# benlevyx/vi-normflows

Hardware: AMD Instinct MI355X
Metric: ELBO samples/sec (whole node), 32-layer RealNVP on 784-dim synthetic (higher is better)
Workload: dtype bf16; 1 GPU; model=RealNVP-32 VI, 784-d, conditioner 392-1024-1024-784, 72.2M params, global_batch=65536, dim=784, parallelism=dp1

## Files before the change

csrc/bindings/gemm_ops.cpp:

```cpp
#include <vector>
#include <torch/library.h>
#include <ATen/ATen.h>

#include <cstdlib>

#include "bind_common.h"
#include "launchers.h"
#include "nf_common.h"

namespace {

long ld2(const at::Tensor& t) { return t.size(0) <= 1 ? t.size(1) : t.stride(0); }

void chk_amax_slots(const at::Tensor& t) {
  TORCH_CHECK(t.is_cuda() && t.scalar_type() == at::kFloat && t.is_contiguous() &&
                  t.numel() >= NF_AMAX_SLOTS,
              "amax_cur must hold ", NF_AMAX_SLOTS, " contiguous fp32 slots (ops.fp8.DelayedScale)");
}

void chk_mat(const at::Tensor& t, const char* n, at::ScalarType dt) {
  TORCH_CHECK(t.is_cuda(), n, " must be on the GPU");
  TORCH_CHECK(t.dim() == 2, n, " must be 2-D");
  TORCH_CHECK(t.scalar_type() == dt, n, " dtype ", t.scalar_type(), " expected ", dt);
  TORCH_CHECK(t.size(1) <= 1 || t.stride(1) == 1, n, " needs unit inner stride");
  TORCH_CHECK(ld2(t) % 8 == 0, n, " leading dimension must be a multiple of 8 (16-B rows)");
  TORCH_CHECK(reinterpret_cast<uintptr_t>(t.data_ptr()) % 16 == 0, n, " must be 16-B aligned");
}

void chk_q(const at::Tensor& t, const char* n) {
  TORCH_CHECK(t.is_cuda() && t.dim() == 2, n, " must be a 2-D GPU tensor");
  TORCH_CHECK(t.scalar_type() == at::kByte || t.scalar_type() == at::kFloat8_e4m3fn, n,
              " must be uint8 / float8_e4m3fn");
  TORCH_CHECK(t.stride(1) == 1 && ld2(t) % 16 == 0, n, " rows must be 16-B aligned");
  TORCH_CHECK(reinterpret_cast<uintptr_t>(t.data_ptr()) % 16 == 0, n, " must be 16-B aligned");
}

void chk_ranges(const at::Tensor& r, long ntiles, const char* n);

int64_t gemm_nt(const at::Tensor& x, const at::Tensor& W, const c10::optional<at::Tensor>& b,
                const at::Tensor& y, int64_t relu, const c10::optional<at::Tensor>& mask,
                bool mask_lanes) {
  chk_mat(x, "x", at::kBFloat16);
  chk_mat(W, "W", at::kBFloat16);
  chk_mat(y, "y", at::kBFloat16);
  const int M = x.size(0), K = x.size(1), N = W.size(0);
  TORCH_CHECK(W.size(1) == K, "W inner dim");
  TORCH_CHECK(y.size(0) == M && y.size(1) == N, "y shape");
  TORCH_CHECK(K % 32 == 0, "K must be a multiple of 32 (pad the operands)");
  TORCH_CHECK(N % 8 == 0, "N must be a multiple of 8");
  const void* bp = nullptr;
  if (b && b->defined()) {
    TORCH_CHECK(b->scalar_type() == at::kBFloat16 && b->numel() == N && b->is_contiguous(), "bias");
    bp = b->data_ptr();
  }
  void* mp = nullptr;
  long ldm = 0;
  if (mask && mask->defined()) {
    TORCH_CHECK(mask->is_cuda() && mask->dim() == 2 && mask->scalar_type() == at::kByte &&
                    mask->stride(1) == 1, "mask must be a 2-D uint8 GPU tensor with unit inner stride");
    TORCH_CHECK(relu, "the bitmask records 1(y > 0) of a ReLU layer");
    TORCH_CHECK(mask->size(0) == M && mask->size(1) * 8 == N, "mask shape [M, N/8]");
    TORCH_CHECK(ld2(y) % 8 == 0 && ((uintptr_t)y.data_ptr() & 15) == 0,
                "bitmask output needs 16-B aligned y rows");
    mp = mask->data_ptr();
    ldm = ld2(*mask);
  }
  if (mask_lanes) {
    TORCH_CHECK(mp, "mask_lanes needs a mask");
    if (!mask->is_contiguous()) return NF_LANES_SHAPE;
  }
  return nf_launch_gemm_nt(x.data_ptr(), ld2(x), W.data_ptr(), ld2(W), bp, y.data_ptr(), ld2(y), M,
                           N, K, (int)relu, cur_stream(), mp, ldm, mask_lanes ? 1 : 0);
}

int64_t gemm_mask_lanes_route(int64_t M, int64_t N, int64_t K_fwd, int64_t K_bwd, bool bwd_wt) {
  return nf_gemm_mask_lanes_route((int)M, (int)N, (int)K_fwd, (int)K_bwd, bwd_wt ? 1 : 0);
}

void gemm_nt_f32out(const at::Tensor& x, const at::Tensor& W, const at::Tensor& y) {
  chk_mat(x, "x", at::kBFloat16);
  chk_mat(W, "W", at::kBFloat16);
  chk_mat(y, "y", at::kFloat);
  const int M = x.size(0), K = x.size(1), N = W.size(0);
  TORCH_CHECK(W.size(1) == K, "W inner dim");
  TORCH_CHECK(y.size(0) == M && y.size(1) == N, "y shape");
  TORCH_CHECK(K % 32 == 0 && K > 0, "K must be a positive multiple of 32 (pad the operands)");
  TORCH_CHECK(N % 8 == 0, "N must be a multiple of 8");
  nf_launch_gemm_nt_f32out(x.data_ptr(), ld2(x), W.data_ptr(), ld2(W), y.data_ptr<float>(), ld2(y),
                           M, N, K, cur_stream());
}

void gemm_fp(const at::Tensor& A, bool a_kmajor, const at::Tensor& B, bool b_kmajor,
             const c10::optional<at::Tensor>& bias, const at::Tensor& C, bool accumulate,
             const c10::optional<at::Tensor>& dbias) {
  const auto dt = C.scalar_type();
  TORCH_CHECK(dt == at::kFloat || dt == at::kDouble, "gemm_fp: fp32 or fp64 output");
  auto chk = [&](const at::Tensor& t, const char* n) {
    TORCH_CHECK(t.is_cuda() && t.dim() == 2 && t.scalar_type() == dt, n,
                " must be a 2-D GPU tensor of the output's dtype");
    TORCH_CHECK(t.size(1) <= 1 || t.stride(1) == 1, n, " needs unit inner stride");
  };
  chk(A, "A"); chk(B, "B"); chk(C, "C");
  const int M = C.size(0), N = C.size(1);
  const int K = a_kmajor ? A.size(1) : A.size(0);
  TORCH_CHECK((a_kmajor ? A.size(0) : A.size(1)) == M, "A rows must match C rows");
  TORCH_CHECK((b_kmajor ? B.size(0) : B.size(1)) == N, "B rows must match C cols");
  TORCH_CHECK((b_kmajor ? B.size(1) : B.size(0)) == K, "A / B inner dims differ");
  const void* bp = nullptr;
  if (bias && bias->defined()) {
    TORCH_CHECK(bias->is_cuda() && bias->scalar_type() == dt && bias->is_contiguous() &&
                    bias->numel() == N, "bias: contiguous [N] of the output's dtype");
    bp = bias->data_ptr();
  }
  void* dbp = nullptr;
  if (dbias && dbias->defined()) {
    TORCH_CHECK(dbias->is_cuda() && dbias->scalar_type() == dt && dbias->is_contiguous() &&
                    dbias->numel() == M, "dbias: contiguous [M] of the output's dtype");
    dbp = dbias->data_ptr();
  }
  auto ld = [](const at::Tensor& t) { return t.size(0) <= 1 ? t.size(1) : t.stride(0); };
  const int S = nf_gemm_fp_splits(M, N, K);
  at::Tensor work;
  if (S > 1) work = at::empty({(long)S * ((long)M * N + M)}, C.options());
  nf_launch_gemm_fp(dt == at::kDouble, A.data_ptr(), ld(A), a_kmajor, B.data_ptr(), ld(B),
                    b_kmajor, bp, C.data_ptr(), ld(C), dbp, M, N, K, accumulate, cur_stream(),
                    S > 1 ? work.data_ptr() : nullptr, S);
}

int64_t gemm_nn(const at::Tensor& dy, const at::Tensor& W, const c10::optional<at::Tensor>& h,
                const at::Tensor& dx, bool accumulate, const c10::optional<at::Tensor>& hbits,
                const c10::optional<at::Tensor>& Wt, bool hbits_lanes) {
  chk_mat(dy, "dy", at::kBFloat16);
  chk_mat(W, "W", at::kBFloat16);
  const bool f32 = dx.scalar_type() == at::kFloat;
  chk_mat(dx, "dx", f32 ? at::kFloat : at::kBFloat16);
  const int M = dy.size(0), K = dy.size(1), N = W.size(1);
  TORCH_CHECK(W.size(0) == K, "W rows must equal dy cols");
  const bool use_wt = Wt && Wt->defined();
  if (use_wt) {
    chk_mat(*Wt, "Wt", at::kBFloat16);
    TORCH_CHECK(Wt->size(0) == N && Wt->size(1) == K, "Wt must be W^T [N, K]");
    TORCH_CHECK(!f32 && !accumulate, "the transposed-weight path writes bf16");
    TORCH_CHECK(ld2(*Wt) % 8 == 0 && ((uintptr_t)Wt->data_ptr() & 15) == 0, "Wt rows 16-B");
  }
  TORCH_CHECK(dx.size(0) == M && dx.size(1) == N, "dx shape");
  TORCH_CHECK(K % 32 == 0 && N % 8 == 0, "K % 32 and N % 8 required");
  const void* hp = nullptr;
  long ldh = 0;
  if (h && h->defined()) {
    TORCH_CHECK(!f32, "ReLU-mask epilogue writes bf16");
    chk_mat(*h, "h", at::kBFloat16);
    TORCH_CHECK(h->size(0) == M && h->size(1) == N, "h shape");
    hp = h->data_ptr();
    ldh = ld2(*h);
  }
  int bits = 0;
  if (hbits && hbits->defined()) {
    TORCH_CHECK(!hp, "pass either h or hbits");
    TORCH_CHECK(!f32, "ReLU-mask epilogue writes bf16");
    TORCH_CHECK(hbits->is_cuda() && hbits->dim() == 2 && hbits->scalar_type() == at::kByte &&
                    hbits->stride(1) == 1, "hbits must be a 2-D uint8 GPU tensor with unit inner stride");
    TORCH_CHECK(hbits->size(0) == M && hbits->size(1) * 8 == N, "hbits shape [M, N/8]");
    hp = hbits->data_ptr();
    ldh = ld2(*hbits);
    bits = 1;
    if (hbits_lanes) {
      if (!hbits->is_contiguous()) return NF_LANES_SHAPE;
      bits = 2;
    }
  }
  TORCH_CHECK(!hbits_lanes || bits, "hbits_lanes needs hbits");
  TORCH_CHECK(!accumulate || f32, "accumulate needs an fp32 output");
  if (use_wt)
    return nf_launch_gemm256_nt_dgrad(dy.data_ptr(), ld2(dy), Wt->data_ptr(), ld2(*Wt), hp, ldh,
                                      bits, dx.data_ptr(), ld2(dx), M, N, K, cur_stream());
  return nf_launch_gemm_nn(dy.data_ptr(), ld2(dy), W.data_ptr(), ld2(W), hp, ldh, dx.data_ptr(),
                           ld2(dx), f32, accumulate, M, N, K, cur_stream(), bits);
}

void transpose_bf16_batched(const at::Tensor& desc, int64_t n, int64_t tiles) {
  TORCH_CHECK(desc.is_cuda() && desc.scalar_type() == at::kLong && desc.is_contiguous() &&
                  desc.numel() >= 5 * n, "desc: int64 GPU [n, 5]");
  nf_launch_transpose_bf16_batched(desc.data_ptr(), (int)n, (int)tiles, cur_stream());
}

void gemm_tn(const at::Tensor& dy, const at::Tensor& x, const at::Tensor& dW,
             const c10::optional<at::Tensor>& db) {
  chk_mat(dy, "dy", at::kBFloat16);
  chk_mat(x, "x", at::kBFloat16);
  chk_mat(dW, "dW", at::kFloat);
  const int K = dy.size(0), M = dy.size(1), N = x.size(1);
  TORCH_CHECK(x.size(0) == K, "batch mismatch");
  TORCH_CHECK(dW.size(0) == M && dW.size(1) == N, "dW shape");
  TORCH_CHECK(K % 32 == 0 && M % 8 == 0 && N % 8 == 0, "K % 32, M % 8, N % 8 required");
  float* dbp = nullptr;
  if (db && db->defined()) {
    TORCH_CHECK(db->scalar_type() == at::kFloat && db->numel() == M && db->is_contiguous(), "db");
    dbp = db->data_ptr<float>();
  }
  const int splits = nf_gemm_tn_splits(M, N, K);
  at::Tensor work;
  float* wp = nullptr;
  const long ws = nf_gemm_tn_workspace(M, N, splits);
  if (ws > 0) {
    work = at::empty({ws}, dW.options());
    wp = work.data_ptr<float>();
  }
  nf_launch_gemm_tn(dy.data_ptr(), ld2(dy), x.data_ptr(), ld2(x), dW.data_ptr<float>(), ld2(dW), dbp,
                    M, N, K, splits, wp, cur_stream());
}

void gemm_tn_group(at::TensorList dy, at::TensorList x, at::TensorList dW,
                   const c10::List<c10::optional<at::Tensor>>& db,
                   const c10::List<c10::optional<at::Tensor>>& skip,
                   const c10::List<c10::optional<at::Tensor>>& cmask) {
  const size_t n = dy.size();
  TORCH_CHECK(n >= 1 && n <= 4 && x.size() == n && dW.size() == n && db.size() == n,
              "gemm_tn_group: 1..4 problems with matching lists");
  NfTnProblem pr[4];
  for (size_t p = 0; p < n; ++p) {
    chk_mat(dy[p], "dy", at::kBFloat16);
    chk_mat(x[p], "x", at::kBFloat16);
    chk_mat(dW[p], "dW", at::kFloat);
    const int K = dy[p].size(0), M = dy[p].size(1), N = x[p].size(1);
    TORCH_CHECK(x[p].size(0) == K, "batch mismatch");
    TORCH_CHECK(dW[p].size(0) == M && dW[p].size(1) == N, "dW shape");
    TORCH_CHECK(K % 32 == 0 && M % 8 == 0 && N % 8 == 0, "K % 32, M % 8, N % 8 required");
    float* dbp = nullptr;
    const c10::optional<at::Tensor> b = db.get(p);
    if (b && b->defined()) {
      TORCH_CHECK(b->scalar_type() == at::kFloat && b->numel() == M && b->is_contiguous(), "db");
      dbp = b->data_ptr<float>();
    }
    pr[p] = NfTnProblem{dy[p].data_ptr(), ld2(dy[p]), x[p].data_ptr(), ld2(x[p]),
                        dW[p].data_ptr<float>(), ld2(dW[p]), dbp, M, N, K};
    if (skip.size() == n) {
      const c10::optional<at::Tensor> sk = skip.get(p);
      if (sk && sk->defined()) {
        TORCH_CHECK(sk->is_cuda() && sk->scalar_type() == at::kByte && sk->is_contiguous() &&
                        sk->numel() == (long)((M + 127) / 128) * ((N + 127) / 128), "skip flags");
        pr[p].skip = sk->data_ptr<uint8_t>();
      }
    }
    if (cmask.size() == n) {
      const c10::optional<at::Tensor> cm = cmask.get(p);
      if (cm && cm->defined()) {
        TORCH_CHECK(cm->is_cuda() && cm->scalar_type() == at::kByte && cm->is_contiguous() &&
                        cm->numel() == (long)M * N && N % 4 == 0, "cmask [M,N] uint8");
        TORCH_CHECK(ld2(dW[p]) == N, "cmask needs a dense dW");
        pr[p].cmask = cm->data_ptr<uint8_t>();
      }
    }
  }
  at::Tensor work;
  float* wp = nullptr;
  const long ws = nf_gemm_tn_group_workspace((int)n, pr);
  if (ws > 0) {
    work = at::empty({ws}, dW[0].options());
    wp = work.data_ptr<float>();
  }
  nf_launch_gemm_tn_group((int)n, pr, wp, cur_stream());
}

static void gemm_tn_multi_impl(at::TensorList dy, at::TensorList x, at::TensorList dW,
                               const c10::List<c10::optional<at::Tensor>>& db, int64_t tile0,
                               int64_t ntiles, const c10::List<c10::optional<at::Tensor>>& tiles,
                               const c10::List<c10::optional<at::Tensor>>& cmask,
                               const at::Tensor* f8_scales, at::IntArrayRef sa_idx,
                               at::IntArrayRef sb_idx, int layout = 0) {
  const size_t n = dy.size();
  TORCH_CHECK(layout >= 0 && layout <= 4 && (layout == 0 || !f8_scales), "layout 0..4, bf16");
  const bool f8 = f8_scales != nullptr;
  const auto odt = f8 ? at::kFloat8_e4m3fn : at::kBFloat16;
  if (f8) {
    TORCH_CHECK(f8_scales->is_cuda() && f8_scales->scalar_type() == at::kFloat &&
                    f8_scales->is_contiguous() && sa_idx.size() == n && sb_idx.size() == n,
                "gemm_tn_multi_f8: fp32 scale pool and one (sa, sb) index pair per problem");
    for (size_t p = 0; p < n; ++p)
      TORCH_CHECK(sa_idx[p] >= 0 && sb_idx[p] >= 0 && sa_idx[p] < f8_scales->numel() &&
                      sb_idx[p] < f8_scales->numel() && sa_idx[p] <= 0xffff &&
                      sb_idx[p] <= 0x7fff,
                  "gemm_tn_multi_f8: scale index outside the pool");
  }
  TORCH_CHECK(n >= 1 && n <= 40 && x.size() == n && dW.size() == n && db.size() == n,
              "gemm_tn_multi: 1..40 problems with matching lists");
  TORCH_CHECK((tiles.size() == 0 || tiles.size() == n) && (cmask.size() == 0 || cmask.size() == n),
              "gemm_tn_multi: tiles / cmask lists must be empty or one entry per problem");
  std::vector<NfTnProblem> pr(n);
  long total = 0;
  for (size_t p = 0; p < n; ++p) {
    chk_mat(dy[p], "dy", odt);
    chk_mat(x[p], "x", odt);
    chk_mat(dW[p], "dW", at::kFloat);
    const int K = layout == 2 ? dy[p].size(1) : dy[p].size(0);
    const int M = layout == 2 ? dy[p].size(0) : dy[p].size(1);
    const int N = layout == 1 ? x[p].size(0) : x[p].size(1);
    TORCH_CHECK((layout == 1 ? x[p].size(1) : x[p].size(0)) == K, "batch mismatch");
    TORCH_CHECK(dW[p].size(0) == M && dW[p].size(1) == N, "dW shape");
    TORCH_CHECK(K % 32 == 0 && M % 8 == 0 && N % 8 == 0, "K % 32, M % 8, N % 8 required");
    TORCH_CHECK(!f8 || (K % 128 == 0 && M % 16 == 0 && N % 16 == 0 && ld2(dy[p]) % 16 == 0 &&
                        ld2(x[p]) % 16 == 0 && ld2(dW[p]) % 4 == 0 &&
                        ((uintptr_t)dW[p].data_ptr() & 15) == 0),
                "gemm_tn_multi_f8: K % 128, M / N / ld % 16, 16-B aligned dW");
    TORCH_CHECK(ld2(dy[p]) < (1L << 31) && ld2(x[p]) < (1L << 31) && ld2(dW[p]) < (1L << 31),
                "leading dimensions must fit in int32");
    float* dbp = nullptr;
    const c10::optional<at::Tensor> b = db.get(p);
    if (b && b->defined()) {
      TORCH_CHECK(b->scalar_type() == at::kFloat && b->numel() == M && b->is_contiguous(), "db");
      dbp = b->data_ptr<float>();
    }
    pr[p] = NfTnProblem{dy[p].data_ptr(), ld2(dy[p]), x[p].data_ptr(), ld2(x[p]),
                        dW[p].data_ptr<float>(), ld2(dW[p]), dbp, M, N, K};
    if (f8) {
      pr[p].sa_idx = (int)sa_idx[p];
      pr[p].sb_idx = (int)sb_idx[p];
    }
    int nt = nf_gemm256_tiles(M, N);
    if (tiles.size() == n) {
      const c10::optional<at::Tensor> tl = tiles.get(p);
      if (tl && tl->defined()) {
        TORCH_CHECK(tl->is_cuda() && tl->scalar_type() == at::kShort && tl->is_contiguous() &&
                        tl->numel() >= 1 && tl->numel() <= nt,
                    "tiles: int16 GPU list of active 256x256 tile ids");
        pr[p].tiles = reinterpret_cast<const unsigned short*>(tl->data_ptr<int16_t>());
        pr[p].ntiles_active = nt = (int)tl->numel();
      }
    }
    if (cmask.size() == n) {
      const c10::optional<at::Tensor> cm = cmask.get(p);
      if (cm && cm->defined()) {
        TORCH_CHECK(cm->is_cuda() && cm->scalar_type() == at::kByte && cm->is_contiguous() &&
                        cm->numel() == (long)M * N && ld2(dW[p]) == N, "cmask [M,N] uint8, dense dW");
        pr[p].cmask = cm->data_ptr<uint8_t>();
      }
    }
    total += nt;
  }
  TORCH_CHECK(tile0 >= 0 && ntiles >= 1 && tile0 + ntiles <= total, "tile range outside the ",
              total, " tiles of the problem list");
  nf_launch_gemm256_tn_multi((int)n, pr.data(), (int)tile0, (int)ntiles, cur_stream(),
                             f8 ? f8_scales->data_ptr<float>() : nullptr, layout);
}

void gemm_tn_multi_layout(at::TensorList dy, at::TensorList x, at::TensorList dW,
                          const c10::List<c10::optional<at::Tensor>>& db, int64_t tile0,
                          int64_t ntiles, int64_t layout) {
  const c10::List<c10::optional<at::Tensor>> none;
  gemm_tn_multi_impl(dy, x, dW, db, tile0, ntiles, none, none, nullptr, {}, {}, (int)layout);
}

void gemm_tn_multi(at::TensorList dy, at::TensorList x, at::TensorList dW,
                   const c10::List<c10::optional<at::Tensor>>& db, int64_t tile0, int64_t ntiles,
                   const c10::List<c10::optional<at::Tensor>>& tiles,
                   const c10::List<c10::optional<at::Tensor>>& cmask) {
  gemm_tn_multi_impl(dy, x, dW, db, tile0, ntiles, tiles, cmask, nullptr, {}, {});
}

void gemm_tn_multi_f8(at::TensorList dy, at::TensorList x, at::TensorList dW,
                      const c10::List<c10::optional<at::Tensor>>& db, int64_t tile0,
                      int64_t ntiles, const c10::List<c10::optional<at::Tensor>>& tiles,
                      const c10::List<c10::optional<at::Tensor>>& cmask, const at::Tensor& scales,
                      at::IntArrayRef sa_idx, at::IntArrayRef sb_idx) {
  gemm_tn_multi_impl(dy, x, dW, db, tile0, ntiles, tiles, cmask, &scales, sa_idx, sb_idx);
}

void fp8_colsum(at::TensorList q, at::TensorList out, const at::Tensor& scales,
                at::IntArrayRef sidx, const at::Tensor& part) {
  const size_t n = q.size();
  TORCH_CHECK(n >= 1 && n <= 40 && out.size() == n && sidx.size() == n,
              "fp8_colsum: 1..40 tensors with matching lists");
  TORCH_CHECK(scales.is_cuda() && scales.scalar_type() == at::kFloat && scales.is_contiguous(),
              "fp8_colsum: fp32 scale pool");
  std::vector<const void*> qp(n);
  std::vector<long> ld(n);
  std::vector<int> K(n), N(n), si(n);
  std::vector<float*> op(n);
  for (size_t i = 0; i < n; ++i) {
    chk_mat(q[i], "q", at::kFloat8_e4m3fn);
    K[i] = (int)q[i].size(0);
    N[i] = (int)q[i].size(1);
    TORCH_CHECK(out[i].is_cuda() && out[i].scalar_type() == at::kFloat && out[i].is_contiguous() &&
                    out[i].numel() == N[i], "fp8_colsum: out[i] fp32 [N]");
    TORCH_CHECK(sidx[i] >= 0 && sidx[i] < scales.numel(), "fp8_colsum: scale index");
    qp[i] = q[i].data_ptr();
    ld[i] = ld2(q[i]);
    op[i] = out[i].data_ptr<float>();
    si[i] = (int)sidx[i];
  }
  TORCH_CHECK(part.is_cuda() && part.scalar_type() == at::kFloat && part.is_contiguous() &&
                  part.numel() >= nf_fp8_colsum_workspace((int)n, N.data()),
              "fp8_colsum: part workspace too small");
  nf_launch_fp8_colsum((int)n, qp.data(), ld.data(), K.data(), N.data(), op.data(), si.data(),
                       scales.data_ptr<float>(), part.data_ptr<float>(), cur_stream());
}

void gemm_nt_cpl(const at::Tensor& h, const at::Tensor& W, const c10::optional<at::Tensor>& b,
                 const c10::optional<at::Tensor>& st_opt, const at::Tensor& x, const at::Tensor& y,
                 const c10::optional<at::Tensor>& yb, const at::Tensor& ldjp, bool ldj_init,
                 double scale, bool inverse) {
  chk_mat(h, "h", at::kBFloat16);
  chk_mat(W, "W", at::kBFloat16);
  const int M = h.size(0), K = h.size(1), Dh = x.size(1);
  const bool has_st = st_opt && st_opt->defined();
  TORCH_CHECK(has_st || inverse, "st (s_hat output) is required in the forward");
  if (has_st) {
    chk_mat(*st_opt, "st", at::kBFloat16);
    TORCH_CHECK(st_opt->size(0) == M && st_opt->size(1) >= Dh, "st shape");
  }
  TORCH_CHECK(W.size(1) == K && W.size(0) >= 2 * Dh, "W: [>= 2 Dh, K]");
  TORCH_CHECK(K % 32 == 0 && Dh % 8 == 0, "K % 32 and Dh % 8 required");
  for (const at::Tensor* t : {&x, &y})
    TORCH_CHECK(t->is_cuda() && t->scalar_type() == at::kFloat && t->dim() == 2 &&
                    t->stride(1) == 1 && t->size(0) == M && t->size(1) == Dh &&
                    ld2(*t) % 4 == 0 && reinterpret_cast<uintptr_t>(t->data_ptr()) % 16 == 0,
                "x, y: fp32 [M, Dh], 16-B aligned rows");
  const int ntn = (Dh + 127) / 128;
  TORCH_CHECK(ldjp.is_cuda() && ldjp.scalar_type() == at::kFloat && ldjp.dim() == 2 &&
                  ldjp.size(0) >= ntn && ldjp.size(1) == M && ldjp.stride(1) == 1,
              "ldjp: fp32 [ceil(Dh/128), M]");
  const void* bp = nullptr;
  if (b && b->defined()) {
    TORCH_CHECK(b->scalar_type() == at::kBFloat16 && b->numel() == W.size(0) && b->is_contiguous(),
                "bias");
    bp = b->data_ptr();
  }
  void* ybp = nullptr;
  long ldyb = 0;
  int ybw = 0;
  if (yb && yb->defined()) {
    chk_mat(*yb, "yb", at::kBFloat16);
    TORCH_CHECK(yb->size(0) == M && yb->size(1) >= Dh && yb->size(1) % 8 == 0, "yb shape");
    ybp = yb->data_ptr();
    ldyb = ld2(*yb);
    ybw = (int)yb->size(1);
  }
  nf_launch_gemm256_nt_cpl(h.data_ptr(), ld2(h), W.data_ptr(), ld2(W), (int)W.size(0), bp,
                           has_st ? st_opt->data_ptr() : nullptr, has_st ? ld2(*st_opt) : 0, M,
                           K, Dh, x.data_ptr<float>(), ld2(x), y.data_ptr<float>(), ld2(y), ybp,
                           ldyb, ybw, ldjp.data_ptr<float>(), ldjp.stride(0), ldj_init,
                           (float)scale, cur_stream(), inverse ? 1 : 0);
}

void gemm_nn_cpl(const at::Tensor& dy, const at::Tensor& W, const at::Tensor& G,
                 const at::Tensor& s_hat, const at::Tensor& x, const at::Tensor& dst,
                 const at::Tensor& gx, double scale, double c, const c10::optional<at::Tensor>& Wt) {
  chk_mat(dy, "dy", at::kBFloat16);
  chk_mat(W, "W", at::kBFloat16);
  const int M = dy.size(0), K = dy.size(1), N = W.size(1);
  TORCH_CHECK(W.size(0) == K, "W rows must equal dy cols");
  const bool use_wt = Wt && Wt->defined();
  if (use_wt) {
    chk_mat(*Wt, "Wt", at::kBFloat16);
    TORCH_CHECK(Wt->size(0) == N && Wt->size(1) == K, "Wt must be W^T [N, K]");
    TORCH_CHECK(ld2(*Wt) % 8 == 0 && ((uintptr_t)Wt->data_ptr() & 15) == 0, "Wt rows 16-B");
  }
  TORCH_CHECK(K % 32 == 0 && N % 8 == 0, "K % 32 and N % 8 required");
  for (const at::Tensor* t : {&G, &s_hat, &x, &dst, &gx})
    TORCH_CHECK(t->is_cuda() && t->dim() == 2 && t->stride(1) == 1 && t->size(0) == M,
                "gemm_nn_cpl: 2-D GPU operands with unit inner stride and M rows");
  const int Dh = x.size(1);
  const bool x_bf16 = x.scalar_type() == at::kBFloat16;
  const bool g_bf16 = G.scalar_type() == at::kBFloat16, gx_bf16 = gx.scalar_type() == at::kBFloat16;
  TORCH_CHECK((G.scalar_type() == at::kFloat || (g_bf16 && x_bf16)) && G.size(1) == N,
              "G: fp32 (or bf16 with bf16 x) [M, N]");
  TORCH_CHECK((x.scalar_type() == at::kFloat || (x_bf16 && use_wt)) &&
                  (gx.scalar_type() == at::kFloat || (gx_bf16 && x_bf16)) && gx.size(1) == Dh,
              "x: fp32 (or bf16 with Wt) [M, Dh], gx: fp32 (or bf16 with bf16 x) [M, Dh]");
  TORCH_CHECK(s_hat.scalar_type() == at::kBFloat16 && s_hat.size(1) >= Dh, "s_hat: bf16 [M, >= Dh]");
  TORCH_CHECK(dst.scalar_type() == at::kBFloat16 && dst.size(1) >= 2 * Dh && dst.size(1) <= Dh + N,
              "dst: bf16 [M, 2 Dh .. Dh + N]");
  auto al = [](const at::Tensor& t, uintptr_t a) {
    return reinterpret_cast<uintptr_t>(t.data_ptr()) % a == 0;
  };
  TORCH_CHECK(Dh % 4 == 0 && N % 4 == 0 && ld2(G) % 4 == 0 && ld2(x) % 4 == 0 &&
                  ld2(gx) % 4 == 0 && ld2(dst) % 4 == 0 && ld2(s_hat) % 4 == 0,
              "gemm_nn_cpl: Dh, N and every leading dimension must be multiples of 4");
  TORCH_CHECK(al(G, g_bf16 ? 8 : 16) && al(x, x_bf16 ? 8 : 16) && al(gx, gx_bf16 ? 8 : 16) &&
                  al(dst, 8) && al(s_hat, 8),
              "gemm_nn_cpl: G / x / gx must be 16-B aligned (8-B as bf16), dst / s_hat 8-B aligned");
  nf_launch_gemm256_nn_cpl(dy.data_ptr(), ld2(dy), use_wt ? Wt->data_ptr() : W.data_ptr(),
                           use_wt ? ld2(*Wt) : ld2(W), (const float*)G.data_ptr(),
                           ld2(G), M, N, K, s_hat.data_ptr(), ld2(s_hat), (const float*)x.data_ptr(),
                           ld2(x), dst.data_ptr(), ld2(dst), (int)dst.size(1),
                           (float*)gx.data_ptr(), ld2(gx), Dh, (float)scale, (float)c, cur_stream(),
                           use_wt ? 1 : 0, nullptr, 1, 0, nullptr, x_bf16 ? 1 : 0, g_bf16 ? 1 : 0,
                           gx_bf16 ? 1 : 0);
}

void maf_gemm_fwd(const at::Tensor& h, const c10::optional<at::Tensor>& hs, const at::Tensor& W,
                  const c10::optional<at::Tensor>& ws, const c10::optional<at::Tensor>& b,
                  const at::Tensor& krange, const at::Tensor& s_out, const at::Tensor& x,
                  const c10::optional<at::Tensor>& u, const c10::optional<at::Tensor>& ubf,
                  const at::Tensor& ldjp,
                  bool ldj_init, double bound, const c10::optional<at::Tensor>& uq,
                  const c10::optional<at::Tensor>& q_amax_prev,
                  const c10::optional<at::Tensor>& q_scale,
                  const c10::optional<at::Tensor>& q_amax_cur) {
  const bool f8 = h.scalar_type() != at::kBFloat16;
  if (f8) {
    chk_q(h, "h");
    chk_q(W, "W");
    TORCH_CHECK(hs && hs->defined() && ws && ws->defined(), "fp8 operands need hs and ws");
    TORCH_CHECK(hs->is_cuda() && hs->scalar_type() == at::kFloat && hs->numel() >= 1, "hs");
    TORCH_CHECK(ws->is_cuda() && ws->scalar_type() == at::kFloat && ws->is_contiguous() &&
                    ws->numel() == W.size(0), "ws: fp32 [2D]");
  } else {
    chk_mat(h, "h", at::kBFloat16);
    chk_mat(W, "W", at::kBFloat16);
  }
  chk_mat(s_out, "s_out", at::kBFloat16);
  const bool x_bf16 = x.scalar_type() == at::kBFloat16;
  chk_mat(x, "x", x_bf16 ? at::kBFloat16 : at::kFloat);
  const bool has_u = u && u->defined();
  if (has_u) chk_mat(*u, "u", at::kFloat);
  TORCH_CHECK(has_u || (ubf && ubf->defined()),
              "maf_gemm_fwd: u may be omitted only with a ubf output (a bf16 state)");
  const int M = h.size(0), K = h.size(1), D = x.size(1);
  TORCH_CHECK(W.size(0) == 2 * D && W.size(1) == K, "W must be [2D, K]");
  TORCH_CHECK(K % (f8 ? 128 : 32) == 0, "maf_gemm_fwd: K must be a multiple of 32 (e4m3: 128)");
  TORCH_CHECK(D % 128 == 0 && x.size(0) == M && (!has_u || (u->size(0) == M && u->size(1) == D)) &&
                  s_out.size(0) == M && s_out.size(1) == D, "maf_gemm_fwd shapes (D % 128 == 0)");
  chk_ranges(krange, D / 128, "krange");
  TORCH_CHECK(ldjp.is_cuda() && ldjp.scalar_type() == at::kFloat && ldjp.dim() == 2 &&
                  ldjp.size(0) >= D / 128 && ldjp.size(1) == M && ldjp.stride(1) == 1,
              "ldjp: fp32 [D/128, M]");
  const void* bp = nullptr;
  if (b && b->defined()) {
    TORCH_CHECK(b->scalar_type() == at::kBFloat16 && b->numel() == 2 * D && b->is_contiguous(),
                "b: bf16 [2D]");
    bp = b->data_ptr();
  }
  void* ubp = nullptr;
  long ldub = 0;
  if (ubf && ubf->defined()) {
    chk_mat(*ubf, "ubf", at::kBFloat16);
    TORCH_CHECK(ubf->size(0) == M && ubf->size(1) == D, "ubf shape");
    ubp = ubf->data_ptr();
    ldub = ld2(*ubf);
  }
  void* qp = nullptr;
  long ldq = 0;
  const float* qap = nullptr;
  float* qs = nullptr;
  float* qac = nullptr;
  if (uq && uq->defined()) {
    TORCH_CHECK(f8, "the e4m3 copy of u belongs to the fp8 path");
    chk_q(*uq, "uq");
    TORCH_CHECK(uq->size(0) == M && uq->size(1) == D, "uq shape");
    TORCH_CHECK(q_amax_prev && q_scale && q_amax_cur, "uq needs the delayed-scale state");
    chk_amax_slots(*q_amax_cur);
    qp = uq->data_ptr();
    ldq = ld2(*uq);
    qap = q_amax_prev->data_ptr<float>();
    qs = q_scale->data_ptr<float>();
    qac = q_amax_cur->data_ptr<float>();
  }
  nf_launch_gemm256_maf_fwd(h.data_ptr(), ld2(h), f8 ? 1 : 0, f8 ? hs->data_ptr<float>() : nullptr,
                            W.data_ptr(), ld2(W), f8 ? ws->data_ptr<float>() : nullptr, bp,
                            krange.data_ptr<int>(), s_out.data_ptr(), ld2(s_out), M, K, D,
                            (const float*)x.data_ptr(), ld2(x),
                            has_u ? u->data_ptr<float>() : nullptr, has_u ? ld2(*u) : 0, ubp, ldub,
                            ldjp.data_ptr<float>(), ldjp.stride(0), ldj_init, (float)bound, qp, ldq,
                            qap, qs, qac, cur_stream(), x_bf16 ? 1 : 0);
}

struct F8Out {
  void* q = nullptr;
  long ldq = 0;
  const float* ap = nullptr;
  float* qs = nullptr;
  float* ac = nullptr;
};
F8Out f8_out(const c10::optional<at::Tensor>& q, const c10::optional<at::Tensor>& amax_prev,
             const c10::optional<at::Tensor>& scale, const c10::optional<at::Tensor>& amax_cur,
             long rows, long cols) {
  F8Out o;
  if (!(q && q->defined())) return o;
  chk_q(*q, "q");
  TORCH_CHECK(q->size(0) == rows && q->size(1) == cols, "e4m3 copy shape");
  TORCH_CHECK(amax_prev && scale && amax_cur && amax_prev->defined() && scale->defined() &&
                  amax_cur->defined(), "the e4m3 copy needs the delayed-scale state");
  chk_amax_slots(*amax_cur);
  o.q = q->data_ptr();
  o.ldq = ld2(*q);
  o.ap = amax_prev->data_ptr<float>();
  o.qs = scale->data_ptr<float>();
  o.ac = amax_cur->data_ptr<float>();
  return o;
}

void chk_scales(const c10::optional<at::Tensor>& sa, const c10::optional<at::Tensor>& sb,
                long nb) {
  TORCH_CHECK(sa && sa->defined() && sb && sb->defined(), "fp8 operands need sa and sb");
  TORCH_CHECK(sa->is_cuda() && sa->scalar_type() == at::kFloat && sa->numel() >= 1, "sa");
  TORCH_CHECK(sb->is_cuda() && sb->scalar_type() == at::kFloat && sb->is_contiguous() &&
                  sb->numel() == nb && ((uintptr_t)sb->data_ptr() & 15) == 0,
              "sb: fp32 per-row scales, 16-B aligned");
}

void fp8_dgrad(const at::Tensor& dyq, const at::Tensor& sa, const at::Tensor& Wtq,
               const at::Tensor& sb, const at::Tensor& h, const c10::optional<at::Tensor>& dx_opt,
               const at::Tensor& krange256, const c10::optional<at::Tensor>& dxq,
               const c10::optional<at::Tensor>& q_amax_prev,
               const c10::optional<at::Tensor>& q_scale,
               const c10::optional<at::Tensor>& q_amax_cur) {
  chk_q(dyq, "dyq");
  chk_q(Wtq, "Wtq");
  const int M = dyq.size(0), K = dyq.size(1), N = Wtq.size(0);
  TORCH_CHECK(Wtq.size(1) == K && K % 128 == 0 && N % 8 == 0, "Wtq [N, K], K % 128 == 0");
  const bool h_bits = h.scalar_type() == at::kByte;
  if (h_bits) {
    TORCH_CHECK(h.is_cuda() && h.dim() == 2 && h.size(0) == M && h.size(1) * 8 >= N &&
                    h.stride(1) == 1, "h bitmask: uint8 [M, N/8]");
  } else {
    chk_mat(h, "h", at::kBFloat16);
  }
  TORCH_CHECK(h.size(0) == M && (h_bits || h.size(1) == N), "h");
  const bool has_dx = dx_opt && dx_opt->defined();
  TORCH_CHECK(has_dx || (dxq && dxq->defined()), "fp8_dgrad: dx and / or dxq");
  if (has_dx) {
    chk_mat(*dx_opt, "dx", at::kBFloat16);
    TORCH_CHECK(dx_opt->size(0) == M && dx_opt->size(1) == N, "dx");
  }
  chk_scales(sa, sb, N);
  const long nt = (N + 255) / 256;
  const int segs = krange256.numel() == 4 * nt ? 2 : 1;
  chk_ranges(krange256, segs * nt, "krange256");
  const F8Out o = f8_out(dxq, q_amax_prev, q_scale, q_amax_cur, M, N);
  nf_launch_gemm256_fp8_dgrad(dyq.data_ptr(), ld2(dyq), sa.data_ptr<float>(), Wtq.data_ptr(),
                              ld2(Wtq), sb.data_ptr<float>(), h.data_ptr(), ld2(h), h_bits ? 1 : 0,
                              has_dx ? dx_opt->data_ptr() : nullptr, has_dx ? ld2(*dx_opt) : N,
                              M, N, K, krange256.data_ptr<int>(), segs,
                              o.q, o.ldq, o.ap, o.qs, o.ac, cur_stream());
}

void maf_gemm_bwd(const at::Tensor& dy, const at::Tensor& Wt, const at::Tensor& krange256,
                  const at::Tensor& G, const at::Tensor& s_raw, const at::Tensor& u,
                  const c10::optional<at::Tensor>& dst_opt, const at::Tensor& gx, double bound,
                  double c,
                  const c10::optional<at::Tensor>& sa, const c10::optional<at::Tensor>& sb,
                  const c10::optional<at::Tensor>& dstq,
                  const c10::optional<at::Tensor>& q_amax_prev,
                  const c10::optional<at::Tensor>& q_scale,
                  const c10::optional<at::Tensor>& q_amax_cur) {
  const bool f8 = dy.scalar_type() != at::kBFloat16;
  if (f8) {
    chk_q(dy, "dy");
    chk_q(Wt, "Wt");
    chk_scales(sa, sb, Wt.size(0));
  } else {
    chk_mat(dy, "dy", at::kBFloat16);
    chk_mat(Wt, "Wt", at::kBFloat16);
    TORCH_CHECK(!(dstq && dstq->defined()), "the e4m3 copy of dst belongs to the fp8 path");
  }
  chk_mat(s_raw, "s_raw", at::kBFloat16);
  const bool has_dst = dst_opt && dst_opt->defined();
  TORCH_CHECK(has_dst || (f8 && dstq && dstq->defined()), "maf_gemm_bwd: dst and / or dstq");
  if (has_dst) chk_mat(*dst_opt, "dst", at::kBFloat16);
  chk_mat(G, "G", at::kFloat);
  const bool u_bf16 = u.scalar_type() == at::kBFloat16;
  chk_mat(u, "u", u_bf16 ? at::kBFloat16 : at::kFloat);
  chk_mat(gx, "gx", at::kFloat);
  const int M = dy.size(0), K = dy.size(1), D = Wt.size(0);
  TORCH_CHECK(Wt.size(1) == K && K % 32 == 0 && D % 8 == 0, "Wt must be [D, K], K % 32 == 0");
  TORCH_CHECK(!f8 || K % 128 == 0, "maf_gemm_bwd: e4m3 operands need K % 128 == 0");
  for (const at::Tensor* t : {&G, &s_raw, &u, &gx})
    TORCH_CHECK(t->size(0) == M && t->size(1) == D, "G / s_raw / u / gx: [M, D]");
  TORCH_CHECK(!has_dst || (dst_opt->size(0) == M && dst_opt->size(1) == 2 * D),
              "dst: bf16 [M, 2D]");
  const long nt = (D + 255) / 256;
  const int segs = krange256.numel() == 4 * nt ? 2 : 1;
  chk_ranges(krange256, segs * nt, "krange256");
  NfF8Operands fo{};
  if (f8) {
    const F8Out o = f8_out(dstq, q_amax_prev, q_scale, q_amax_cur, M, 2 * D);
    fo.sa = sa->data_ptr<float>();
    fo.sb = sb->data_ptr<float>();
    fo.q = o.q; fo.ldq = o.ldq;
    fo.q_amax_prev = o.ap; fo.q_scale_out = o.qs; fo.q_amax_cur = o.ac;
  }
  nf_launch_gemm256_nn_cpl(dy.data_ptr(), ld2(dy), Wt.data_ptr(), ld2(Wt), G.data_ptr<float>(),
                           ld2(G), M, D, K, s_raw.data_ptr(), ld2(s_raw),
                           (const float*)u.data_ptr(), ld2(u),
                           has_dst ? dst_opt->data_ptr() : nullptr,
                           has_dst ? ld2(*dst_opt) : 2 * D, 2 * D, gx.data_ptr<float>(), ld2(gx),
                           D, (float)bound, (float)c, cur_stream(), 1, krange256.data_ptr<int>(),
                           segs, 1, f8 ? &fo : nullptr, u_bf16 ? 1 : 0);
}

void fp8_quant_rows_strided(const at::Tensor& x, int64_t layer_stride, int64_t rows_per,
                            int64_t layers, int64_t C, const at::Tensor& q, const at::Tensor& scale) {
  TORCH_CHECK(x.is_cuda() && (x.scalar_type() == at::kFloat || x.scalar_type() == at::kBFloat16) &&
                  x.is_contiguous(), "x fp32 / bf16 GPU");
  TORCH_CHECK(x.numel() >= (layers - 1) * layer_stride + rows_per * C, "x too small");
  chk_q(q, "q");
  TORCH_CHECK(q.size(0) == rows_per * layers && q.size(1) >= C && q.size(1) % 4 == 0, "q shape");
  TORCH_CHECK(scale.is_cuda() && scale.scalar_type() == at::kFloat &&
                  scale.numel() == rows_per * layers, "scale");
  nf_launch_fp8_quant_rows_strided(x.data_ptr(), x.scalar_type() == at::kBFloat16, C,
                                   layer_stride, (int)rows_per,
                                   (int)(rows_per * layers), (int)C, q.data_ptr(), ld2(q), q.size(1),
                                   scale.data_ptr<float>(), cur_stream());
}

void maf_fwd(const at::Tensor& x, const at::Tensor& o, double bound, const at::Tensor& u,
             const c10::optional<at::Tensor>& ubf, const c10::optional<at::Tensor>& uq,
             const c10::optional<at::Tensor>& amax_prev, const c10::optional<at::Tensor>& scale,
             const c10::optional<at::Tensor>& amax_cur, const at::Tensor& ldj, bool ldj_init) {
  chk_mat(x, "x", at::kFloat);
  chk_mat(o, "o", at::kBFloat16);
  chk_mat(u, "u", at::kFloat);
  const int B = x.size(0), D = x.size(1);
  TORCH_CHECK(D % 4 == 0 && o.size(0) == B && o.size(1) == 2 * D && u.size(0) == B && u.size(1) == D,
              "maf_fwd shapes");
  TORCH_CHECK(ldj.is_cuda() && ldj.scalar_type() == at::kFloat && ldj.numel() == B, "ldj");
  void* ub = nullptr;
  long ldub = 0;
  if (ubf && ubf->defined()) {
    chk_mat(*ubf, "ubf", at::kBFloat16);
    ub = ubf->data_ptr();
    ldub = ld2(*ubf);
  }
  void* q = nullptr;
  long ldq = 0;
  const float* ap = nullptr;
  float* sc = nullptr;
  float* ac = nullptr;
  if (uq && uq->defined()) {
    chk_q(*uq, "uq");
    TORCH_CHECK(amax_prev && scale && amax_cur, "fp8 output needs the delayed-scale state");
    q = uq->data_ptr();
    ldq = ld2(*uq);
    ap = amax_prev->data_ptr<float>();
    sc = scale->data_ptr<float>();
    ac = amax_cur->data_ptr<float>();
    chk_amax_slots(*amax_cur);
  }
  nf_launch_maf_fwd(x.data_ptr<float>(), ld2(x), o.data_ptr(), ld2(o), B, D, (float)bound,
                    u.data_ptr<float>(), ld2(u), ub, ldub, q, ldq, ap, sc, ac,
                    ldj.data_ptr<float>(), ldj_init, cur_stream());
}

void maf_bwd(const at::Tensor& gu, const at::Tensor& u, const at::Tensor& o, double bound,
             double c_ldj, const at::Tensor& dout, const at::Tensor& gx,
             const c10::optional<at::Tensor>& c_row) {
  chk_mat(gu, "gu", at::kFloat);
  chk_mat(u, "u", at::kFloat);
  chk_mat(o, "o", at::kBFloat16);
  chk_mat(dout, "dout", at::kBFloat16);
  chk_mat(gx, "gx", at::kFloat);
  const int B = gu.size(0), D = gu.size(1);
  TORCH_CHECK(D % 4 == 0 && u.size(0) == B && u.size(1) == D && o.size(0) == B &&
                  (o.size(1) == 2 * D || o.size(1) == D) && dout.size(1) == 2 * D &&
                  gx.size(1) == D, "maf_bwd shapes");
  const void* sp = static_cast<const at::BFloat16*>(o.data_ptr()) + (o.size(1) == 2 * D ? D : 0);
  const float* cr = nullptr;
  if (c_row && c_row->defined()) {
    TORCH_CHECK(c_row->is_cuda() && c_row->scalar_type() == at::kFloat &&
                    c_row->is_contiguous() && c_row->numel() == B, "c_row: fp32 [B]");
    cr = c_row->data_ptr<float>();
  }
  nf_launch_maf_bwd(gu.data_ptr<float>(), ld2(gu), u.data_ptr<float>(), ld2(u), sp,
                    ld2(o), B, D, (float)bound, (float)c_ldj, dout.data_ptr(), ld2(dout),
                    gx.data_ptr<float>(), ld2(gx), cur_stream(), cr);
}

void iaf_gate_fwd(const at::Tensor& o, const at::Tensor& z, double gate_bias, const at::Tensor& y,
                  const at::Tensor& ldj, const c10::optional<at::Tensor>& ybf) {
  chk_mat(o, "o", at::kBFloat16);
  chk_mat(z, "z", at::kFloat);
  chk_mat(y, "y", at::kFloat);
  const int B = z.size(0), D = z.size(1);
  TORCH_CHECK(D % 4 == 0 && o.size(0) == B && o.size(1) == 2 * D && y.size(0) == B &&
                  y.size(1) == D, "iaf_gate_fwd shapes");
  TORCH_CHECK(ldj.is_cuda() && ldj.scalar_type() == at::kFloat && ldj.is_contiguous() &&
                  ldj.numel() == B, "ldj: fp32 [B]");
  void* yb = nullptr;
  long ldyb = 0;
  if (ybf && ybf->defined()) {
    chk_mat(*ybf, "ybf", at::kBFloat16);
    TORCH_CHECK(ybf->size(0) == B && ybf->size(1) == D && ld2(*ybf) % 4 == 0 &&
                    reinterpret_cast<uintptr_t>(ybf->data_ptr()) % 8 == 0,
                "ybf: bf16 [B, D], 8-B aligned rows");
    yb = ybf->data_ptr();
    ldyb = ld2(*ybf);
  }
  nf_launch_iaf_gate_fwd(o.data_ptr(), ld2(o), z.data_ptr<float>(), ld2(z), B, D, (float)gate_bias,
                         y.data_ptr<float>(), ld2(y), ldj.data_ptr<float>(), cur_stream(), yb,
                         ldyb);
}

void iaf_gate_bwd(const at::Tensor& gy, const c10::optional<at::Tensor>& gl, const at::Tensor& z,
                  const at::Tensor& o, double gate_bias, const at::Tensor& dout,
                  const at::Tensor& gz) {
  chk_mat(gy, "gy", at::kFloat);
  chk_mat(z, "z", at::kFloat);
  chk_mat(o, "o", at::kBFloat16);
  chk_mat(dout, "dout", at::kBFloat16);
  chk_mat(gz, "gz", at::kFloat);
  const int B = z.size(0), D = z.size(1);
  TORCH_CHECK(D % 4 == 0 && gy.size(0) == B && gy.size(1) == D && o.size(0) == B &&
                  o.size(1) == 2 * D && dout.size(0) == B && dout.size(1) == 2 * D &&
                  gz.size(0) == B && gz.size(1) == D, "iaf_gate_bwd shapes");
  const float* glp = nullptr;
  if (gl && gl->defined()) {
    TORCH_CHECK(gl->is_cuda() && gl->scalar_type() == at::kFloat && gl->is_contiguous() &&
                    gl->numel() == B, "gl: fp32 [B]");
    glp = gl->data_ptr<float>();
  }
  nf_launch_iaf_gate_bwd(gy.data_ptr<float>(), ld2(gy), glp, z.data_ptr<float>(), ld2(z),
                         o.data_ptr(), ld2(o), B, D, (float)gate_bias, dout.data_ptr(), ld2(dout),
                         gz.data_ptr<float>(), ld2(gz), cur_stream());
}

void chk_ranges(const at::Tensor& r, long ntiles, const char* n) {
  TORCH_CHECK(r.is_cuda() && r.scalar_type() == at::kInt && r.is_contiguous() && r.numel() == 2 * ntiles,
              n, " must be an int32 GPU tensor [n_tiles, 2]");
}

void masked_gemm_nt(const at::Tensor& x, const at::Tensor& W, const c10::optional<at::Tensor>& b,
                    const at::Tensor& y, int64_t relu, const at::Tensor& krange,
                    const c10::optional<at::Tensor>& krange256) {
  chk_mat(x, "x", at::kBFloat16);
  chk_mat(W, "W", at::kBFloat16);
  chk_mat(y, "y", at::kBFloat16);
  const int M = x.size(0), K = x.size(1), N = W.size(0);
  TORCH_CHECK(W.size(1) == K && y.size(0) == M && y.size(1) == N, "shapes");
  TORCH_CHECK(K % 32 == 0 && N % 8 == 0, "K % 32 and N % 8 required");
  chk_ranges(krange, (N + 127) / 128, "krange");
  const void* bp = (b && b->defined()) ? b->data_ptr() : nullptr;
  const int* k256 = nullptr;
  if (krange256 && krange256->defined()) {
    chk_ranges(*krange256, (N + 255) / 256, "krange256");
    k256 = krange256->data_ptr<int>();
  }
  nf_launch_gemm_nt_masked(x.data_ptr(), ld2(x), W.data_ptr(), ld2(W), bp, y.data_ptr(), ld2(y), M,
                           N, K, (int)relu, krange.data_ptr<int>(), cur_stream(), k256);
}

void masked_gemm_nn(const at::Tensor& dy, const at::Tensor& W, const c10::optional<at::Tensor>& h,
                    const at::Tensor& dx, const at::Tensor& krange, bool accumulate,
                    const c10::optional<at::Tensor>& krange256, const c10::optional<at::Tensor>& Wt) {
  chk_mat(dy, "dy", at::kBFloat16);
  chk_mat(W, "W", at::kBFloat16);
  const bool f32 = dx.scalar_type() == at::kFloat;
  chk_mat(dx, "dx", f32 ? at::kFloat : at::kBFloat16);
  const int M = dy.size(0), K = dy.size(1), N = W.size(1);
  TORCH_CHECK(W.size(0) == K && dx.size(0) == M && dx.size(1) == N, "shapes");
  TORCH_CHECK(K % 32 == 0 && N % 8 == 0, "K % 32 and N % 8 required");
  chk_ranges(krange, (N + 127) / 128, "krange");
  const void* hp = nullptr;
  long ldh = 0;
  if (h && h->defined()) {
    chk_mat(*h, "h", at::kBFloat16);
    hp = h->data_ptr();
    ldh = ld2(*h);
  }
  TORCH_CHECK(!accumulate || f32, "accumulate needs an fp32 dx");
  const int* k256 = nullptr;
  int segs = 1;
  if (krange256 && krange256->defined()) {
    const long nt = (N + 255) / 256;
    segs = krange256->numel() == 4 * nt ? 2 : 1;
    chk_ranges(*krange256, segs * nt, "krange256");
    TORCH_CHECK(!hp || (ld2(*h) % 8 == 0 && ((uintptr_t)hp & 15) == 0),
                "ReLU-mask operand rows must be 16-B aligned for the 256x256 kernel");
    k256 = krange256->data_ptr<int>();
  }
  const void* wtp = nullptr;
  long ldwt = 0;
  if (Wt && Wt->defined()) {
    chk_mat(*Wt, "Wt", at::kBFloat16);
    TORCH_CHECK(Wt->size(0) == N && Wt->size(1) == K, "Wt must be W^T [N, K]");
    TORCH_CHECK(ld2(*Wt) % 8 == 0 && ((uintptr_t)Wt->data_ptr() & 15) == 0, "Wt rows 16-B");
    wtp = Wt->data_ptr();
    ldwt = ld2(*Wt);
  }
  nf_launch_gemm_nn_masked(dy.data_ptr(), ld2(dy), W.data_ptr(), ld2(W), hp, ldh, dx.data_ptr(),
                           ld2(dx), f32, accumulate, M, N, K, krange.data_ptr<int>(), cur_stream(),
                           k256, segs, wtp, ldwt);
}

void masked_gemm_tn(const at::Tensor& dy, const at::Tensor& x, const at::Tensor& dW,
                    const c10::optional<at::Tensor>& db, const at::Tensor& skip) {
  chk_mat(dy, "dy", at::kBFloat16);
  chk_mat(x, "x", at::kBFloat16);
  chk_mat(dW, "dW", at::kFloat);
  const int K = dy.size(0), M = dy.size(1), N = x.size(1);
  TORCH_CHECK(x.size(0) == K && dW.size(0) == M && dW.size(1) == N, "shapes");
  TORCH_CHECK(K % 32 == 0 && M % 8 == 0 && N % 8 == 0, "K % 32, M % 8, N % 8 required");
  TORCH_CHECK(skip.is_cuda() && skip.scalar_type() == at::kByte && skip.is_contiguous() &&
                  skip.numel() == (long)((M + 127) / 128) * ((N + 127) / 128),
              "skip must be a uint8 GPU tensor [tiles]");
  float* dbp = (db && db->defined()) ? db->data_ptr<float>() : nullptr;
  const int splits = nf_gemm_tn_splits(M, N, K);
  at::Tensor work;
  float* wp = nullptr;
  const long ws = nf_gemm_tn_workspace(M, N, splits);
  if (ws > 0) {
    work = at::empty({ws}, dW.options());
    wp = work.data_ptr<float>();
  }
  nf_launch_gemm_tn_masked(dy.data_ptr(), ld2(dy), x.data_ptr(), ld2(x), dW.data_ptr<float>(),
                           ld2(dW), dbp, M, N, K, splits, wp, skip.data_ptr<unsigned char>(),
                           cur_stream());
}

}


void fp8_quant_rows(const at::Tensor& x, const at::Tensor& q, const at::Tensor& scale) {
  TORCH_CHECK(x.is_cuda() && x.dim() == 2 && x.stride(1) == 1, "x: 2-D GPU, unit inner stride");
  TORCH_CHECK(x.scalar_type() == at::kBFloat16 || x.scalar_type() == at::kFloat, "x bf16/fp32");
  chk_q(q, "q");
  TORCH_CHECK(q.size(0) == x.size(0) && q.size(1) >= x.size(1) && q.size(1) % 4 == 0, "q shape");
  TORCH_CHECK(scale.is_cuda() && scale.scalar_type() == at::kFloat && scale.numel() == x.size(0) &&
                  scale.is_contiguous(), "scale [rows] fp32");
  nf_launch_fp8_quant_rows(x.data_ptr(), x.scalar_type() == at::kBFloat16, ld2(x), x.size(0),
                           x.size(1), q.data_ptr(), ld2(q), q.size(1), scale.data_ptr<float>(),
                           cur_stream());
}

void fp8_quant_tensor(const at::Tensor& x, const at::Tensor& q, const at::Tensor& amax_prev,
                      const at::Tensor& scale, const at::Tensor& amax_cur) {
  TORCH_CHECK(x.is_cuda() && x.dim() == 2 && x.stride(1) == 1, "x: 2-D GPU, unit inner stride");
  TORCH_CHECK(x.scalar_type() == at::kBFloat16 || x.scalar_type() == at::kFloat, "x bf16/fp32");
  chk_q(q, "q");
  TORCH_CHECK(q.size(0) == x.size(0) && q.size(1) >= x.size(1) && q.size(1) % 4 == 0, "q shape");
  for (const at::Tensor* t : {&amax_prev, &scale, &amax_cur})
    TORCH_CHECK(t->is_cuda() && t->scalar_type() == at::kFloat && t->numel() >= 1, "scalars fp32");
  chk_amax_slots(amax_cur);
  nf_launch_fp8_quant_tensor(x.data_ptr(), x.scalar_type() == at::kBFloat16, ld2(x), x.size(0),
                             x.size(1), q.data_ptr(), ld2(q), q.size(1), amax_prev.data_ptr<float>(),
                             scale.data_ptr<float>(), amax_cur.data_ptr<float>(), cur_stream());
}

void gemm_fp8_nt(const at::Tensor& xq, const at::Tensor& sx, const at::Tensor& wq,
                 const at::Tensor& sw, const c10::optional<at::Tensor>& b,
                 const c10::optional<at::Tensor>& y_opt, int64_t relu,
                 const c10::optional<at::Tensor>& krange,
                 const c10::optional<at::Tensor>& yq, const c10::optional<at::Tensor>& q_amax_prev,
                 const c10::optional<at::Tensor>& q_scale, const c10::optional<at::Tensor>& q_amax_cur,
                 const c10::optional<at::Tensor>& krange256,
                 const c10::optional<at::Tensor>& mask_out) {
  chk_q(xq, "xq");
  chk_q(wq, "wq");
  const bool has_y = y_opt && y_opt->defined();
  const bool has_mask = mask_out && mask_out->defined();
  const int M = xq.size(0), K = xq.size(1), N = wq.size(0);
  TORCH_CHECK(wq.size(1) == K, "shapes");
  if (has_y) {
    chk_mat(*y_opt, "y", at::kBFloat16);
    TORCH_CHECK(y_opt->size(0) == M && y_opt->size(1) == N, "y shape");
  }
  TORCH_CHECK(has_y || (yq && yq->defined()) || has_mask, "gemm_fp8_nt: no output");
  if (has_mask) {
    TORCH_CHECK(mask_out->is_cuda() && mask_out->scalar_type() == at::kByte && mask_out->dim() == 2 &&
                    mask_out->size(0) == M && mask_out->size(1) * 8 >= N && mask_out->stride(1) == 1 &&
                    relu, "mask_out: uint8 [M, N/8] bitmask of a ReLU product");
  }
  TORCH_CHECK(K % 128 == 0 && N % 8 == 0, "K % 128 and N % 8 required");
  TORCH_CHECK(sx.is_cuda() && sx.scalar_type() == at::kFloat && (sx.numel() == M || sx.numel() == 1) &&
                  sx.is_contiguous(), "sx [M] or [1]");
  TORCH_CHECK(sw.is_cuda() && sw.scalar_type() == at::kFloat && sw.numel() == N && sw.is_contiguous(), "sw");
  const void* bp = nullptr;
  if (b && b->defined()) {
    TORCH_CHECK(b->scalar_type() == at::kBFloat16 && b->numel() == N && b->is_contiguous(), "bias");
    bp = b->data_ptr();
  }
  const int* kr = nullptr;
  if (krange && krange->defined()) {
    chk_ranges(*krange, (N + 127) / 128, "krange");
    kr = krange->data_ptr<int>();
  }
  void* qp = nullptr;
  long ldq = 0;
  const float* qap = nullptr;
  float* qs = nullptr;
  float* qac = nullptr;
  if (yq && yq->defined()) {
    chk_q(*yq, "yq");
    TORCH_CHECK(yq->size(0) == M && yq->size(1) == N, "yq shape");
    TORCH_CHECK(q_amax_prev && q_scale && q_amax_cur, "yq needs the delayed-scale state");
    qp = yq->data_ptr();
    ldq = ld2(*yq);
    qap = q_amax_prev->data_ptr<float>();
    qs = q_scale->data_ptr<float>();
    qac = q_amax_cur->data_ptr<float>();
    chk_amax_slots(*q_amax_cur);
  }
  const bool dense = !(krange && krange->defined());
  const bool has256 = krange256 && krange256->defined();
  const long ldy = has_y ? ld2(*y_opt) : N;
  const bool lean = !has_y || has_mask;
  if ((dense || has256) && (lean || nf_gemm_prefer_256(M, N, K)) && ld2(xq) % 16 == 0 &&
      ld2(wq) % 16 == 0 && ldy % 8 == 0 && (!qp || ldq % 8 == 0)) {
    const int* k256 = nullptr;
    if (has256) {
      chk_ranges(*krange256, (N + 255) / 256, "krange256");
      k256 = krange256->data_ptr<int>();
    }
    nf_launch_gemm256_fp8_nt(xq.data_ptr(), ld2(xq), sx.data_ptr<float>(),
                             sx.numel() == M && M > 1, wq.data_ptr(), ld2(wq), sw.data_ptr<float>(),
                             bp, has_y ? y_opt->data_ptr() : nullptr, ldy, M, N, K, (int)relu,
                             k256, qp, ldq, qap, qs, qac, cur_stream(),
                             has_mask ? mask_out->data_ptr<uint8_t>() : nullptr,
                             has_mask ? ld2(*mask_out) : 0);
    return;
  }
  TORCH_CHECK(!lean, "gemm_fp8_nt: y-less / bitmask forms need the 256 kernel (krange256, 16-B rows)");
  nf_launch_gemm_fp8_nt(xq.data_ptr(), ld2(xq), sx.data_ptr<float>(), sx.numel() == M && M > 1,
                        wq.data_ptr(), ld2(wq),
                        sw.data_ptr<float>(), bp, y_opt->data_ptr(), ldy, M, N, K, (int)relu, kr,
                        qp, ldq, qap, qs, qac, cur_stream());
}

int64_t gemm_set_mode(int64_t mode) { return nf_gemm_set_mode((int)mode); }
int64_t gemm_pair(int64_t mode) { return nf_gemm256_set_pair((int)mode); }
int nf_gemm_cpl4w(int on);
int64_t gemm_cpl4w(int64_t on) { return nf_gemm_cpl4w((int)on); }
int nf_gemm256_xcd_pack(int on);
int64_t gemm_wgrad_xcd_pack(int64_t on) { return nf_gemm256_xcd_pack((int)on); }
int64_t gemm_persist(int64_t on) {
  const int prev = nf_gemm256_get_persist();
  if (on >= 0) nf_gemm256_set_persist((int)on);
  return prev;
}
int64_t gemm_grid_reserve(int64_t cus) {
  return nf_gemm256_set_reserve((int)cus);
}
#ifdef NF_G256_STAMPS
void nf_g256_set_stamps(void* p);
void g256_set_stamps(const at::Tensor& buf) { nf_g256_set_stamps(buf.numel() ? buf.data_ptr() : nullptr); }
#endif

TORCH_LIBRARY_FRAGMENT(vinf, m) {
#ifdef NF_G256_STAMPS
  m.def("g256_set_stamps(Tensor buf) -> ()", &g256_set_stamps);
#endif
  m.def("gemm_set_mode(int mode) -> int", &gemm_set_mode);
  m.def("gemm_pair(int mode) -> int", &gemm_pair);
  m.def("gemm_cpl4w(int on) -> int", &gemm_cpl4w);
  m.def("gemm_persist(int on) -> int", &gemm_persist);
  m.def("gemm_grid_reserve(int cus) -> int", &gemm_grid_reserve);
  m.def("gemm_wgrad_xcd_pack(int on) -> int", &gemm_wgrad_xcd_pack);
  m.def("fp8_quant_rows(Tensor x, Tensor(a!) q, Tensor(b!) scale) -> ()");
  m.def("fp8_quant_tensor(Tensor x, Tensor(a!) q, Tensor amax_prev, Tensor(b!) scale, Tensor(c!) amax_cur) -> ()");
  m.def("gemm_fp8_nt(Tensor xq, Tensor sx, Tensor wq, Tensor sw, Tensor? b, Tensor(a!)? y, int relu, Tensor? krange, Tensor(b!)? yq=None, Tensor? q_amax_prev=None, Tensor(c!)? q_scale=None, Tensor(d!)? q_amax_cur=None, Tensor? krange256=None, Tensor(e!)? mask_out=None) -> ()");
  m.def("masked_gemm_nt(Tensor x, Tensor W, Tensor? b, Tensor(a!) y, int relu, Tensor krange, Tensor? krange256=None) -> ()");
  m.def("masked_gemm_nn(Tensor dy, Tensor W, Tensor? h, Tensor(a!) dx, Tensor krange, bool accumulate=False, Tensor? krange256=None, Tensor? Wt=None) -> ()");
  m.def("masked_gemm_tn(Tensor dy, Tensor x, Tensor(a!) dW, Tensor(b!)? db, Tensor skip) -> ()");
  m.def("gemm_nt(Tensor x, Tensor W, Tensor? b, Tensor(a!) y, int relu, Tensor(b!)? mask=None, bool mask_lanes=False) -> int");
  m.def("gemm_mask_lanes_route(int M, int N, int K_fwd, int K_bwd, bool bwd_wt) -> int", &gemm_mask_lanes_route);
  m.def("gemm_nt_f32out(Tensor x, Tensor W, Tensor(a!) y) -> ()");
  m.def("gemm_fp(Tensor A, bool a_kmajor, Tensor B, bool b_kmajor, Tensor? bias, Tensor(a!) C, bool accumulate, Tensor(b!)? dbias=None) -> ()");
  m.def("gemm_nn(Tensor dy, Tensor W, Tensor? h, Tensor(a!) dx, bool accumulate, Tensor? hbits=None, Tensor? Wt=None, bool hbits_lanes=False) -> int");
  m.def("transpose_bf16_batched(Tensor desc, int n, int tiles) -> ()");
  m.def("gemm_tn(Tensor dy, Tensor x, Tensor(a!) dW, Tensor(b!)? db) -> ()");
  m.def("gemm_tn_group(Tensor[] dy, Tensor[] x, Tensor(a!)[] dW, Tensor(b!)?[] db, Tensor?[] skip, Tensor?[] cmask) -> ()");
  m.def("gemm_tn_multi(Tensor[] dy, Tensor[] x, Tensor(a!)[] dW, Tensor(b!)?[] db, int tile0, int ntiles, Tensor?[] tiles, Tensor?[] cmask) -> ()");
  m.def("gemm_tn_multi_layout(Tensor[] dy, Tensor[] x, Tensor(a!)[] dW, Tensor(b!)?[] db, int tile0, int ntiles, int layout) -> ()");
  m.def("fp8_colsum(Tensor[] q, Tensor(a!)[] out, Tensor scales, int[] sidx, Tensor(b!) part) -> ()");
  m.def("gemm_tn_multi_f8(Tensor[] dy, Tensor[] x, Tensor(a!)[] dW, Tensor(b!)?[] db, int tile0, int ntiles, Tensor?[] tiles, Tensor?[] cmask, Tensor scales, int[] sa_idx, int[] sb_idx) -> ()");
  m.def("gemm_nt_cpl(Tensor h, Tensor W, Tensor? b, Tensor(a!)? st, Tensor x, Tensor(b!) y, Tensor(c!)? yb, Tensor(d!) ldjp, bool ldj_init, float scale, bool inverse=False) -> ()");
  m.def("gemm_nn_cpl(Tensor dy, Tensor W, Tensor G, Tensor s_hat, Tensor x, Tensor(a!) dst, Tensor(b!) gx, float scale, float c, Tensor? Wt=None) -> ()");
  m.def("maf_gemm_fwd(Tensor h, Tensor? hs, Tensor W, Tensor? ws, Tensor? b, Tensor krange, Tensor(a!) s_out, Tensor x, Tensor(b!)? u, Tensor(c!)? ubf, Tensor(d!) ldjp, bool ldj_init, float bound, Tensor(e!)? uq=None, Tensor? q_amax_prev=None, Tensor(f!)? q_scale=None, Tensor(g!)? q_amax_cur=None) -> ()");
  m.def("maf_gemm_bwd(Tensor dy, Tensor Wt, Tensor krange256, Tensor G, Tensor s_raw, Tensor u, Tensor(a!)? dst, Tensor(b!) gx, float bound, float c, Tensor? sa=None, Tensor? sb=None, Tensor(c!)? dstq=None, Tensor? q_amax_prev=None, Tensor(d!)? q_scale=None, Tensor(e!)? q_amax_cur=None) -> ()");
  m.def("fp8_dgrad(Tensor dyq, Tensor sa, Tensor Wtq, Tensor sb, Tensor h, Tensor(a!)? dx, Tensor krange256, Tensor(b!)? dxq=None, Tensor? q_amax_prev=None, Tensor(c!)? q_scale=None, Tensor(d!)? q_amax_cur=None) -> ()");
  m.def("fp8_quant_rows_strided(Tensor x, int layer_stride, int rows_per, int layers, int C, Tensor(a!) q, Tensor(b!) scale) -> ()");
  m.def("maf_fwd(Tensor x, Tensor o, float bound, Tensor(a!) u, Tensor(b!)? ubf, Tensor(c!)? uq, Tensor? amax_prev, Tensor(d!)? scale, Tensor(e!)? amax_cur, Tensor(f!) ldj, bool ldj_init) -> ()");
  m.def("iaf_gate_fwd(Tensor o, Tensor z, float gate_bias, Tensor(a!) y, Tensor(b!) ldj, "
        "Tensor(c!)? ybf=None) -> ()");
  m.def("iaf_gate_bwd(Tensor gy, Tensor? gl, Tensor z, Tensor o, float gate_bias, Tensor(a!) dout, Tensor(b!) gz) -> ()");
  m.def("maf_bwd(Tensor gu, Tensor u, Tensor o, float bound, float c_ldj, Tensor(a!) dout, Tensor(b!) gx, Tensor? c_row=None) -> ()");
}

TORCH_LIBRARY_IMPL(vinf, CUDA, m) {
  m.impl("masked_gemm_nt", &masked_gemm_nt);
  m.impl("masked_gemm_nn", &masked_gemm_nn);
  m.impl("masked_gemm_tn", &masked_gemm_tn);
  m.impl("gemm_nt", &gemm_nt);
  m.impl("gemm_nt_f32out", &gemm_nt_f32out);
  m.impl("gemm_fp", &gemm_fp);
  m.impl("gemm_nn", &gemm_nn);
  m.impl("transpose_bf16_batched", &transpose_bf16_batched);
  m.impl("gemm_tn", &gemm_tn);
  m.impl("gemm_tn_group", &gemm_tn_group);
  m.impl("gemm_tn_multi", &gemm_tn_multi);
  m.impl("gemm_tn_multi_f8", &gemm_tn_multi_f8);
  m.impl("fp8_colsum", &fp8_colsum);
  m.impl("gemm_tn_multi_layout", &gemm_tn_multi_layout);
  m.impl("gemm_nn_cpl", &gemm_nn_cpl);
  m.impl("gemm_nt_cpl", &gemm_nt_cpl);
  m.impl("fp8_quant_rows", &fp8_quant_rows);
  m.impl("fp8_quant_rows_strided", &fp8_quant_rows_strided);
  m.impl("maf_fwd", &maf_fwd);
  m.impl("maf_gemm_fwd", &maf_gemm_fwd);
  m.impl("maf_gemm_bwd", &maf_gemm_bwd);
  m.impl("fp8_dgrad", &fp8_dgrad);
  m.impl("maf_bwd", &maf_bwd);
  m.impl("iaf_gate_fwd", &iaf_gate_fwd);
  m.impl("iaf_gate_bwd", &iaf_gate_bwd);
  m.impl("fp8_quant_tensor", &fp8_quant_tensor);
  m.impl("gemm_fp8_nt", &gemm_fp8_nt);
}
```

csrc/include/launchers.h:

```cpp
#pragma once

#include <hip/hip_runtime.h>
#include <stdint.h>

void nf_throw_hip_error(hipError_t e, const char* expr, const char* file, int line);

void nf_launch_coupling_fwd(const void* st, int st_is_bf16, long ld_st_, const float* x, long ld_x,
                            float* y, long ld_y, void* ybf, int ybf_is_bf16, long ld_yb,
                            float* ssav, long ld_s, float* ldj, int B, int Dh, float scale,
                            int inverse, int ldj_init, int yb_width, hipStream_t stream);
void nf_launch_coupling_bwd(const void* s, int s_is_shat_bf16, long ld_s, const float* gy,
                            long ld_gy, const float* x, long ld_x, float c_scalar,
                            const float* c_row, void* dst, int dst_is_bf16, long ld_dst, float* gx,
                            long ld_gx, int B, int Dh, float scale, int gx_accumulate,
                            int dst_pad_to, hipStream_t stream);

void nf_launch_rqs_fwd(const void* params, int params_is_bf16, const float* x, float* y,
                       float* ldj, int B, int Dh, int K, float bound, int inverse, int ldj_init,
                       hipStream_t stream);
void nf_launch_rqs_bwd(const void* params, int params_is_bf16, const float* x, const float* g_out,
                       const float* g_ldj, void* dparams, float* gx, int B, int Dh, int K,
                       float bound, int inverse, hipStream_t stream);

void nf_launch_dsf_fwd(const void* params, int params_is_bf16, const float* x, float* y,
                       float* ldj, int B, int D, int H, int inverse, int ldj_init,
                       hipStream_t stream);
void nf_launch_dsf_bwd(const void* params, int params_is_bf16, const float* x, const float* g_out,
                       const float* g_ldj, void* dparams, float* gx, int B, int D, int H,
                       int inverse, hipStream_t stream);

struct NfSylParams {
  const float *R1, *R2, *d1, *d2, *b, *V;
  long rs_R1, rs_R2, rs_d1, rs_d2, rs_b, rs_V;
};
struct NfSylGrads {
  float *R1, *R2, *d1, *d2, *b, *V;
  long rs_R1, rs_R2, rs_d1, rs_d2, rs_b, rs_V;
};
void nf_launch_sylvester_fwd(const float* z, const NfSylParams& p, const unsigned char* flips,
                             float* zK, float* ldj, float* saved, int N, int D, int K, int H,
                             hipStream_t stream);
void nf_launch_sylvester_bwd(const float* saved, const NfSylParams& p, const unsigned char* flips,
                             const float* gz, const float* gl, float* dz, const NfSylGrads& g,
                             int N, int D, int K, int H, hipStream_t stream);

int nf_stein_splits(int N, int D, int j_splits);
void nf_launch_stein_svgd(const float* x, long ldx, const float* score, long lds,
                          const float* h_dev, float h_host, int kind, int S, float* phi,
                          float* work, int N, int D, hipStream_t stream);
void nf_launch_stein_ksd(const float* x, long ldx, const float* score, long lds,
                         const float* h_dev, float h_host, int kind, int S, float* rows,
                         float* diag, float* work, int N, int D, hipStream_t stream);

int nf_glm_splits(int B, int N, int D, int n_splits);
void nf_launch_glm_logp_grad(const float* theta, long ldt, const float* X, long ldx,
                             const float* y, const float* prec_dev, float prec_host,
                             int has_prior, int family, float inv_var, float scale, int S,
                             float* logp, float* grad, float* work, int B, int N, int D,
                             hipStream_t stream);

void nf_launch_target_logp_grad(int kind, const float* A, long lda, const float* Bh, long ldb,
                                float* gA, long ldga, float* gB, long ldgb, int grad_accumulate,
                                const float* params, float p0, float p1, float p2, float cst,
                                const float* beta_ptr, float beta_host, float row_weight,
                                const float* logq0, const float* ldj, float* logp_out,
                                float* frow_out, int B, int Dh, hipStream_t stream);
void nf_launch_bernoulli_logits(const void* logits, int is_bf16, long ldl_, const float* x, long ldx,
                                void* dlogits, long ldd, const float* coef_ptr, float coef_host,
                                float* logpx, int B, int P, hipStream_t stream);
void nf_launch_energy2d(int kind, const float* z, long ldz, float* logp, float* grad, long ldg,
                        float gscale, const float* logq0, const float* ldj, const float* beta,
                        float* frow, int B, hipStream_t stream);

void nf_launch_reparam_sample(const float* mu, const float* logvar, uint64_t seed,
                              const int64_t* offset_ptr, int64_t offset_host, uint32_t stream_id,
                              float* z, long ldz, float* eps, long lde, void* zbf, int zbf_is_bf16,
                              long ldzb, int nbf, float* logq0, int B, int D, hipStream_t stream);
void nf_launch_normal_fill(float* out, long n, uint64_t seed, const int64_t* offset_ptr,
                           int64_t offset_host, uint32_t stream_id, hipStream_t stream);
void nf_launch_reparam_grad(const float* g_lo, long ldlo, const float* g_hi, long ldhi,
                            const float* eps, long lde, const float* logvar, float* partial,
                            int npartial, float* gmu, float* glv, int B, int D, int Dl,
                            hipStream_t stream);

void nf_launch_flat_optimizer(int kind, float* p, const float* g, float* m, float* v, void* pbf,
                              long n, float lr, float b1, float b2, float eps, float wd,
                              const float* step_ptr, float step_host, const float* gscale_ptr,
                              float gscale_host, const float* skip_ptr, float warmup,
                              hipStream_t stream);
void nf_launch_cu_hold(int blocks, float usec, hipStream_t stream);
void nf_launch_sumsq_guard(const float* x, long n, float* partial, int npartial, float* out_sumsq,
                           float* out_skip, float* out_scale, float max_norm, float base_scale,
                           hipStream_t stream);

enum { NF_LANES_OK = 0, NF_LANES_SHAPE = 1, NF_LANES_KERNEL = 2 };
int nf_launch_gemm_nt(const void* x, long ldx, const void* W, long ldw, const void* bias, void* y,
                      long ldy, int M, int N, int K, int relu, hipStream_t stream,
                      void* mask_out = nullptr, long ld_mask = 0, int mask_lanes = 0);
int nf_gemm_mask_lanes_route(int M, int N, int K_fwd, int K_bwd, int bwd_wt);
int nf_launch_gemm_nn(const void* dy, long lddy, const void* W, long ldw, const void* aux,
                      long ld_aux, void* dx, long lddx, int dx_is_f32, int accumulate, int M,
                      int N, int K, hipStream_t stream, int aux_is_bits = 0);
void nf_launch_gemm_nt_f32out(const void* x, long ldx, const void* W, long ldw, float* y, long ldy,
                              int M, int N, int K, hipStream_t stream);
int nf_gemm_fp_splits(int M, int N, int K);
void nf_launch_gemm_fp(int is_f64, const void* A, long lda, int a_kmajor, const void* B, long ldb,
                       int b_kmajor, const void* bias, void* C, long ldc, void* dbias, int M, int N,
                       int K, int accumulate, hipStream_t stream, void* work = nullptr,
                       int splits = 1);
void nf_launch_gemm_tn(const void* dy, long lddy, const void* x, long ldx, float* dW, long lddw,
                       float* db, int M, int N, int K, int splits, float* work,
                       hipStream_t stream);
long nf_gemm_tn_workspace(int M, int N, int splits);
struct NfTnProblem {
  const void* dy; long lddy;
  const void* x; long ldx;
  float* dW; long lddw;
  float* db;
  int M, N, K;
  const unsigned char* skip = nullptr;
  const unsigned char* cmask = nullptr;
  const unsigned short* tiles = nullptr;
  int ntiles_active = -1;
  int sa_idx = -1, sb_idx = -1;
};
long nf_gemm_tn_group_workspace(int nprob, const NfTnProblem* pr);
void nf_launch_gemm_tn_group(int nprob, const NfTnProblem* pr, float* work, hipStream_t stream);
int nf_launch_gemm256_nt(const void* x, long ldx, const void* W, long ldw, const void* bias,
                         void* y, long ldy, int M, int N, int K, int relu, hipStream_t stream,
                         void* mask_out = nullptr, long ld_mask = 0,
                         const int* krange = nullptr, int mask_lanes = 0);
int nf_launch_gemm256_nn(const void* dy, long lddy, const void* W, long ldw, const void* aux,
                         long ld_aux, void* dx, long lddx, int dx_is_f32, int accumulate, int M,
                         int N, int K, hipStream_t stream, int aux_is_bits = 0,
                         const int* krange = nullptr, int krange_segs = 1, int w_kmajor = 0);
void nf_gemm256_set_persist(int on);
int nf_gemm256_get_persist();
int nf_gemm256_set_reserve(int cus);
int nf_gemm256_set_pair(int mode);
int nf_launch_gemm256_nt_dgrad(const void* dy, long lddy, const void* Wt, long ldwt,
                               const void* aux, long ld_aux, int aux_is_bits, void* dx,
                               long lddx, int M, int N, int K, hipStream_t stream);
void nf_launch_transpose_bf16_batched(const void* desc, int n, int total_tiles,
                                      hipStream_t stream);
void nf_launch_gemm256_nt_cpl(const void* h, long ldh, const void* W, long ldw, int w_rows,
                              const void* bias, void* st, long ld_st, int M, int K, int Dh,
                              const float* x, long ld_x, float* y, long ld_y, void* yb, long ld_yb,
                              int yb_width, float* ldjp, long ld_ldjp, int ldj_init, float scale,
                              hipStream_t stream, int inverse = 0);
struct NfF8Operands {
  const float* sa;
  const float* sb;
  void* q;
  long ldq;
  const float* q_amax_prev;
  float* q_scale_out;
  float* q_amax_cur;
};
void nf_launch_gemm256_nn_cpl(const void* dy, long lddy, const void* W, long ldw, const float* G,
                              long ldg, int M, int N, int K, const void* s_hat, long ld_s,
                              const float* x, long ld_x, void* dst, long ld_dst, int dst_pad,
                              float* gx, long ld_gx, int Dh, float scale, float c,
                              hipStream_t stream, int w_kmajor = 0, const int* krange = nullptr,
                              int krange_segs = 1, int mode = 0, const NfF8Operands* f8 = nullptr,
                              int x_bf16 = 0, int g_in_bf16 = 0, int gx_bf16 = 0);
void nf_launch_gemm256_fp8_dgrad(const void* dyq, long lddy, const float* sa, const void* wtq,
                                 long ldwt, const float* sb, const void* aux, long ld_aux,
                                 int aux_bits, void* dx, long lddx, int M, int N, int K,
                                 const int* krange, int krange_segs, void* dxq, long lddxq,
                                 const float* q_amax_prev, float* q_scale_out, float* q_amax_cur,
                                 hipStream_t stream);
void nf_launch_gemm256_maf_fwd(const void* h, long ldh, int f8, const float* hs, const void* W,
                               long ldw, const float* ws, const void* bias, const int* krange,
                               void* s_out, long ld_s, int M, int K, int D, const float* x,
                               long ld_x, float* u, long ld_u, void* ubf, long ld_ub, float* ldjp,
                               long ld_ldjp, int ldj_init, float bound, void* uq, long lduq,
                               const float* q_amax_prev, float* q_scale_out, float* q_amax_cur,
                               hipStream_t stream, int x_bf16 = 0);
int nf_launch_gemm256_tn_partials(const void* dy, long lddy, const void* x, long ldx, float* C,
                                  long ldc, long slab_stride, float* dbias, int M, int N, int K,
                                  int splits, hipStream_t stream);
int nf_gemm256_tiles(int M, int N);
void nf_launch_gemm256_tn_multi(int nprob, const NfTnProblem* pr, int tile0, int ntiles,
                                hipStream_t stream, const float* f8_scales = nullptr,
                                int layout = 0);
int nf_gemm_set_mode(int mode);
void nf_launch_fp8_quant_rows(const void* x, int x_is_bf16, long ldx, int R, int C, void* q,
                              long ldq, int Cq, float* scale, hipStream_t stream);
long nf_fp8_colsum_workspace(int n, const int* N);
void nf_launch_fp8_colsum(int n, const void* const* q, const long* ld, const int* K, const int* N,
                          float* const* out, const int* sidx, const float* scales, float* part,
                          hipStream_t stream);
void nf_launch_fp8_quant_tensor(const void* x, int x_is_bf16, long ldx, int R, int C, void* q,
                                long ldq, int Cq, const float* amax_prev, float* scale_out,
                                float* amax_cur, hipStream_t stream);
void nf_launch_gemm_fp8_nt(const void* xq, long ldx, const float* sx, int sx_per_row,
                           const void* wq, long ldw, const float* sw, const void* bias, void* y,
                           long ldy, int M, int N, int K, int relu, const int* krange,
                           void* yq, long ldyq, const float* q_amax_prev, float* q_scale_out,
                           float* q_amax_cur, hipStream_t stream);
int nf_gemm_tn_splits(int M, int N, int K);
bool nf_gemm_prefer_256(int M, int N, int K);
void nf_launch_gemm256_fp8_nt(const void* xq, long ldx, const float* sx, int sx_per_row,
                              const void* wq, long ldw, const float* sw, const void* bias, void* y,
                              long ldy, int M, int N, int K, int relu, const int* krange,
                              void* yq, long ldyq, const float* q_amax_prev, float* q_scale_out,
                              float* q_amax_cur, hipStream_t stream,
                              unsigned char* mask_out = nullptr, long ld_mask = 0);

void nf_launch_planar_fwd(const float* z, const float* W, const float* U, const float* B, float* zK,
                          float* ldj, float* saved, int N, int D, int K, int per_sample,
                          int broadcast, hipStream_t stream);
void nf_launch_planar_bwd(const float* saved, const float* W, const float* U, const float* B,
                          const float* gz, const float* gl, float* dz, float* dW, float* dU,
                          float* dB, int N, int D, int K, int per_sample, int broadcast,
                          hipStream_t stream);
int nf_planar_shared_per(int D);
int nf_planar_shared_blocks(int N);
void nf_launch_planar_bwd_shared(const float* z0, const float* W, const float* U, const float* B,
                                 const float* gz, const float* gl, float* dz, float* dW, float* dU,
                                 float* dB, float* part, int nblk, int N, int D, int K,
                                 int broadcast, hipStream_t stream);
void nf_launch_radial_fwd(const float* z, const float* Z0, const float* AL, const float* BE,
                          float* zK, float* ldj, float* saved, int N, int D, int K,
                          int per_sample, hipStream_t stream);
void nf_launch_radial_bwd(const float* saved, const float* Z0, const float* AL, const float* BE,
                          const float* gz, const float* gl, float* dz, float* dZ0, float* dA,
                          float* dBe, int N, int D, int K, int per_sample, hipStream_t stream);
void nf_launch_planar_inv(const float* y, const float* W, const float* U, const float* B, float* x,
                          float* ldj, float* saved, int N, int D, int K, int per_sample,
                          hipStream_t stream);
void nf_launch_planar_inv_bwd(const float* saved, const float* W, const float* U, const float* B,
                              const float* gx, const float* gl, float* dy, float* dW, float* dU,
                              float* dB, int N, int D, int K, int per_sample, hipStream_t stream);
void nf_launch_radial_inv(const float* y, const float* Z0, const float* AL, const float* BE,
                          float* x, float* ldj, float* saved, int N, int D, int K,
                          int per_sample, hipStream_t stream);
void nf_launch_radial_inv_bwd(const float* saved, const float* Z0, const float* AL,
                              const float* BE, const float* gx, const float* gl, float* dy,
                              float* dZ0, float* dA, float* dBe, int N, int D, int K,
                              int per_sample, hipStream_t stream);

void nf_launch_gemm_nt_masked(const void* x, long ldx, const void* W, long ldw, const void* bias,
                              void* y, long ldy, int M, int N, int K, int relu, const int* krange,
                              hipStream_t stream, const int* krange256 = nullptr);
void nf_launch_gemm_nn_masked(const void* dy, long lddy, const void* W, long ldw, const void* aux,
                              long ld_aux, void* dx, long lddx, int dx_is_f32, int accumulate, int M,
                              int N, int K, const int* krange, hipStream_t stream,
                              const int* krange256 = nullptr, int krange256_segs = 1,
                              const void* Wt = nullptr, long ldwt = 0);
void nf_launch_gemm_tn_masked(const void* dy, long lddy, const void* x, long ldx, float* dW,
                              long lddw, float* db, int M, int N, int K, int splits, float* work,
                              const unsigned char* skip, hipStream_t stream);

void nf_launch_maf_fwd(const float* x, long ldx, const void* o, long ldo, int B, int D, float bound,
                       float* u, long ldu, void* ubf, long ldub, void* uq, long lduq,
                       const float* amax_prev, float* scale_out, float* amax_cur, float* ldj,
                       int ldj_init, hipStream_t stream);
void nf_launch_maf_bwd(const float* gu, long ldg, const float* u, long ldu, const void* s_raw,
                       long lds, int B, int D, float bound, float c_ldj, void* dout, long lddo,
                       float* gx, long ldgx, hipStream_t stream, const float* c_row = nullptr);
void nf_launch_iaf_gate_fwd(const void* o, long ldo, const float* z, long ldz, int B, int D,
                            float gate_bias, float* y, long ldy, float* ldj, hipStream_t stream,
                            void* ybf = nullptr, long ldyb = 0);
void nf_launch_iaf_gate_bwd(const float* gy, long ldg, const float* gl, const float* z, long ldz,
                            const void* o, long ldo, int B, int D, float gate_bias, void* dout,
                            long lddo, float* gz, long ldgz, hipStream_t stream);
void nf_launch_fp8_quant_rows_strided(const void* x, int x_is_bf16, long ldx, long layer_stride,
                                      int rows_per, int R, int C, void* q, long ldq, int Cq,
                                      float* scale, hipStream_t stream);

struct NfVaeParams {
  const float* enc_W[4];
  const float* enc_b[4];
  const float* enc_Wo;
  const float* enc_bo;
  const float* dec_W[4];
  const float* dec_b[4];
  const float* dec_Wo;
  const float* dec_bo;
};
struct NfVaeGrads {
  float* enc_W[4];
  float* enc_b[4];
  float* enc_Wo;
  float* enc_bo;
  float* dec_W[4];
  float* dec_b[4];
  float* dec_Wo;
  float* dec_bo;
};
size_t nf_vae_rows_lds_bytes(int Din, int dz, int K, int De);
void nf_launch_vae_step(const NfVaeParams& prm, const float* x, const float* eps_in, unsigned seed,
                        const long* offset, const float* beta, int B, int Din, int dz, int K,
                        int L, float* ws_eact, float* ws_egrad, float* ws_gphi, float* ws_zk,
                        float* ws_dact, float* ws_dgrad, float* ws_dl, float* frow, float* loss,
                        float* zk_out, float* ldj_out, const NfVaeGrads& grd, hipStream_t stream);

#define NF_MADE_SWEEP_MAX_HIDDEN 4
struct NfMadeSweep {
  const float* W[NF_MADE_SWEEP_MAX_HIDDEN];
  const float* b[NF_MADE_SWEEP_MAX_HIDDEN];
  long ldw[NF_MADE_SWEEP_MAX_HIDDEN];
  const float* Wo;
  long ldo;
  const float* bo;
  const float* v;
  long ldv;
  const float* ctx;
  long ldc;
  const int* perm;
  const int* ubeg;
  float* x;
  long ldx;
  float* ldj;
  int B, D, H, L, kind;
  float param;
};
int nf_made_sweep_rows(int D, int H, int L);
void nf_launch_made_sweep(const NfMadeSweep& s, hipStream_t stream);

int nf_dsf_sweep_rows(int D, int H, int L, int U);
void nf_launch_dsf_sweep(const NfMadeSweep& s, int U, hipStream_t stream);

int nf_rqs_sweep_rows(int D, int H, int L, int K);
void nf_launch_rqs_sweep(const NfMadeSweep& s, int K, float bound, hipStream_t stream);

#define NF_SWEEP_ADJOINT_MAX_P 96
struct NfSweepAdjoint {
  const float* W[NF_MADE_SWEEP_MAX_HIDDEN];
  long ldw[NF_MADE_SWEEP_MAX_HIDDEN];
  const float* h[NF_MADE_SWEEP_MAX_HIDDEN];
  long ldh[NF_MADE_SWEEP_MAX_HIDDEN];
  float* a[NF_MADE_SWEEP_MAX_HIDDEN];
  long lda[NF_MADE_SWEEP_MAX_HIDDEN];
  const float* Wo;
  long ldo;
  const int* perm;
  const int* ubeg;
  const float* gx;
  long ldg;
  const float* d;
  long ldd;
  const float* q;
  const float* c;
  float* pbar;
  float* w;
  long ldwo;
  int B, D, H, L, P;
};
int nf_sweep_adjoint_rows(int D, int H, int L, int P);
void nf_launch_sweep_adjoint(const NfSweepAdjoint& s, hipStream_t stream);

struct NfLuSolve {
  const float* M;
  long ldm;
  const float* y;
  long ldy;
  const int* perm;
  const float* bias;
  float* x;
  long ldx;
  int B, D, mode, transpose;
};
int nf_lu_solve_rows(int D);
void nf_launch_lu_solve(const NfLuSolve& s, hipStream_t stream);
```

csrc/include/tn_multi.h:

```cpp
#pragma once
#include "gemm_tile.h"

namespace nf {
namespace gemm {
namespace g256 {

struct TnDesc {
  const bf16_t* A;
  const bf16_t* B;
  float* C;
  float* db;
  const unsigned short* tiles;
  const unsigned char* cmask;
  int lda, ldb, ldc, M, N, K, start, staged;
  int sidx;
};
constexpr int TN_MULTI_MAX = 40;
constexpr int TN_PERM_MAX = 256;
struct TnMulti {
  TnDesc d[TN_MULTI_MAX];
  int n, tile0, ntiles, use_perm;
  unsigned short perm[TN_PERM_MAX];
  const float* scales;
};
static_assert(sizeof(TnMulti) <= 4096, "TnMulti must fit the 4 KiB kernarg segment");

}


bool launch_tn4w_multi(const g256::TnMulti& t, hipStream_t stream);

}
}
```

csrc/kernels/gemm_tn4w.hip:

```cpp

#include "tn_multi.h"

#include <cstdlib>
#include <type_traits>

namespace nf {
namespace gemm {
namespace tn4w {

constexpr int BM = 256, BN = 256, BK = 64, NTHR = 256;

template <int NPIECE = 16>
__device__ __forceinline__ void stage(const bf16_t* __restrict__ base, long ld, int col0,
                                      int cols_total, int k0, char* dst, int lane) {
  unsigned voff[2];
#pragma unroll
  for (int v = 0; v < 2; ++v) {
    const int kr = v * 8 + (lane >> 4);
    const int lc = (lane & 15) ^ mn_swz(kr);
    int gm = col0 + lc * 8;
    gm = gm < cols_total ? gm : cols_total - 8;
    voff[v] = (unsigned)(((lane >> 4) * ld + gm) * 2);
#ifdef NF_PROBE_DMA_SAMEADDR
    voff[v] = 0;
#endif
  }
  const char* b = (const char*)base + (long)k0 * ld * 2;
#pragma unroll
  for (int piece = 0; piece < NPIECE; ++piece) {
#ifdef NF_PROBE_DMA_HALF
    if (piece & 1) continue;
#endif
    const char* row = b + (long)(piece * 4) * ld * 2;
    const unsigned lds = (unsigned)(unsigned long)(LDS_AS char*)(dst + piece * 1024);
    asm volatile("s_mov_b32 m0, %2\n\tglobal_load_lds_dwordx4 %0, %1"
                 :: "v"(voff[(piece >> 1) & 1]), "s"(row), "s"(lds) : "memory", "m0");
  }
}

__device__ __forceinline__ void mfma_acc(v4f& acc, const v8s& a, const v8s& b) {
  asm volatile("v_mfma_f32_16x16x32_bf16 %0, %1, %2, %0" : "+a"(acc) : "v"(a), "v"(b));
}

template <int DBM, int PD>
__device__ __forceinline__ void tile_body4(const GemmArgs& a, int m0, int n0, char* q0, char* q1,
                                           char* q2, char* q3) {
  constexpr int BK4 = 32, HALF4 = 128 * BK4 * 2;
  const int lane = threadIdx.x & 63;
  const int wave = __builtin_amdgcn_readfirstlane(threadIdx.x >> 6);
  const int wr = wave >> 1, wc = wave & 1;
  const int nkt = a.K / BK4;
  const bf16_t* sbase = wave < 2 ? a.A : a.B;
  const long sld = wave < 2 ? a.lda : a.ldb;
  const int scol0 = wave < 2 ? m0 + wave * 128 : n0 + (wave - 2) * 128;
  const int stot = wave < 2 ? a.M : a.N;
  auto stp = [&](auto q_c) -> char* {
    constexpr int Q = decltype(q_c)::value;
    return Q == 0 ? q0 : Q == 1 ? q1 : Q == 2 ? q2 : q3;
  };
  auto issue = [&](int t, auto q_c) {
    stage<8>(sbase, sld, scol0, stot, t * BK4, stp(q_c) + wave * HALF4, lane);
  };
  v4f acc[8][8];
#pragma unroll
  for (int i = 0; i < 8; ++i)
#pragma unroll
    for (int j = 0; j < 8; ++j) acc[i][j] = (v4f){0.f, 0.f, 0.f, 0.f};
  float dbs[8];
#pragma unroll
  for (int j = 0; j < 8; ++j) dbs[j] = 0.f;
  v8s fa[8], fb0[8], fb1[8];
  auto rd_a = [&](auto q_c, int j) { return read_frag<false>(stp(q_c) + wr * HALF4, j * 16, 0, lane); };
  auto rd_b = [&](auto q_c, v8s (&fb)[8]) {
    const char* st = stp(q_c) + (2 + wc) * HALF4;
#pragma unroll
    for (int i = 0; i < 8; ++i) fb[i] = read_frag<false>(st, i * 16, 0, lane);
  };
  v8s* fbn_p = nullptr;
  auto mfma_j = [&](const v8s (&fb)[8], auto qn_c, auto rd_c, auto j_c) {
    constexpr int j = decltype(j_c)::value;
#pragma unroll
    for (int i = 0; i < 8; ++i) mfma_acc(acc[i][j], fb[i], fa[j]);
    if constexpr ((DBM >> j) & 1) {
      typedef __bf16 v2bf __attribute__((ext_vector_type(2)));
      const v2bf one = {(__bf16)1.0f, (__bf16)1.0f};
#pragma unroll
      for (int e = 0; e < 4; ++e) {
        const unsigned w = (unsigned)(unsigned short)fa[j][2 * e] |
                           ((unsigned)(unsigned short)fa[j][2 * e + 1] << 16);
        dbs[j] = __builtin_amdgcn_fdot2_f32_bf16(__builtin_bit_cast(v2bf, w), one, dbs[j], false);
      }
    }
    if constexpr (decltype(rd_c)::value) fa[j] = rd_a(qn_c, j);
    if constexpr (decltype(rd_c)::value && j > 0)
      fbn_p[j] = read_frag<false>(stp(qn_c) + (2 + wc) * HALF4, j * 16, 0, lane);
  };
  auto kstep_from1 = [&](const v8s (&fb)[8], auto qn_c, auto rd_c) {
    mfma_j(fb, qn_c, rd_c, std::integral_constant<int, 1>{});
    mfma_j(fb, qn_c, rd_c, std::integral_constant<int, 2>{});
    mfma_j(fb, qn_c, rd_c, std::integral_constant<int, 3>{});
    mfma_j(fb, qn_c, rd_c, std::integral_constant<int, 4>{});
    mfma_j(fb, qn_c, rd_c, std::integral_constant<int, 5>{});
    mfma_j(fb, qn_c, rd_c, std::integral_constant<int, 6>{});
    mfma_j(fb, qn_c, rd_c, std::integral_constant<int, 7>{});
  };
  using T = std::true_type;
  using F = std::false_type;
  issue(0, std::integral_constant<int, 0>{});
  issue(1, std::integral_constant<int, 1>{});
  if constexpr (PD == 3) {
    issue(2, std::integral_constant<int, 2>{});
    asm volatile("s_waitcnt vmcnt(16)" ::: "memory");
  } else {
    asm volatile("s_waitcnt vmcnt(8)" ::: "memory");
  }
  __builtin_amdgcn_s_barrier();
#pragma unroll
  for (int j = 0; j < 8; ++j) fa[j] = rd_a(std::integral_constant<int, 0>{}, j);
  rd_b(std::integral_constant<int, 0>{}, fb0);
  auto ktile = [&](int t, auto q_c, const v8s (&fbc)[8], v8s (&fbn)[8], auto w2_c, auto next_c,
                   auto issue_c) {
    constexpr int Q = decltype(q_c)::value;
    using QN = std::integral_constant<int, (Q + 1) & 3>;
    using QI = std::integral_constant<int, (Q + PD) & 3>;
    asm volatile("s_waitcnt lgkmcnt(0)" ::: "memory");
    if constexpr (decltype(next_c)::value) {
      if constexpr (PD == 3 && decltype(w2_c)::value) asm volatile("s_waitcnt vmcnt(8)" ::: "memory");
      else asm volatile("s_waitcnt vmcnt(0)" ::: "memory");
    }
    __builtin_amdgcn_sched_barrier(0);
#ifndef NF_PROBE_NOBAR
    __builtin_amdgcn_s_barrier();
#endif
    __builtin_amdgcn_sched_barrier(0);
    mfma_j(fbc, QN{}, next_c, std::integral_constant<int, 0>{});
    __builtin_amdgcn_sched_barrier(0);
#ifndef NF_PROBE_NODMA
    if constexpr (decltype(issue_c)::value) issue(t + PD, QI{});
#endif
    if constexpr (decltype(next_c)::value)
      fbn[0] = read_frag<false>(stp(QN{}) + (2 + wc) * HALF4, 0, 0, lane);
    fbn_p = fbn;
    __builtin_amdgcn_sched_barrier(0);
    kstep_from1(fbc, QN{}, next_c);
  };
  using Q0 = std::integral_constant<int, 0>;
  using Q1 = std::integral_constant<int, 1>;
  using Q2 = std::integral_constant<int, 2>;
  using Q3 = std::integral_constant<int, 3>;
  int t = 0;
  for (; t + 4 < nkt; t += 4) {
    ktile(t, Q0{}, fb0, fb1, T{}, T{}, T{});
    ktile(t + 1, Q1{}, fb1, fb0, T{}, T{}, T{});
    ktile(t + 2, Q2{}, fb0, fb1, T{}, T{}, T{});
    ktile(t + 3, Q3{}, fb1, fb0, T{}, T{}, T{});
  }
  if constexpr (PD == 3) {
    ktile(t, Q0{}, fb0, fb1, T{}, T{}, T{});
    ktile(t + 1, Q1{}, fb1, fb0, T{}, T{}, F{});
  } else {
    ktile(t, Q0{}, fb0, fb1, F{}, T{}, T{});
    ktile(t + 1, Q1{}, fb1, fb0, F{}, T{}, T{});
  }
  ktile(t + 2, Q2{}, fb0, fb1, F{}, T{}, F{});
  ktile(t + 3, Q3{}, fb1, fb0, F{}, F{}, F{});

  const int g = lane >> 4, c = lane & 15;
  if constexpr (DBM != 0) {
#pragma unroll
    for (int j = 0; j < 8; ++j) {
      if (!((DBM >> j) & 1)) continue;
      float v = dbs[j];
      v += __shfl_xor(v, 16);
      v += __shfl_xor(v, 32);
      const int m = m0 + wr * 128 + j * 16 + c;
      if (g == 0 && m < a.M) a.dbias[m] = v;
    }
  }
  __builtin_amdgcn_sched_barrier(0);
  asm volatile("s_nop 7\n\ts_nop 7" ::: "memory");
  __builtin_amdgcn_sched_barrier(0);
  __syncthreads();
  char* region = (wave == 0 ? q0 : wave == 1 ? q1 : wave == 2 ? q2 : q3);
#pragma unroll
  for (int h = 0; h < 2; ++h) {
    v4f sub[4][8];
#pragma unroll
    for (int i = 0; i < 4; ++i)
#pragma unroll
      for (int j = 0; j < 8; ++j) sub[i][j] = acc[4 * h + i][j];
    if (a.staged)
      epi_tile_staged<EPI_F32, 8>(a, sub, m0 + wr * 128, n0 + wc * 128 + h * 64, 0,
                                  region + h * 16384, lane);
    else
#pragma unroll
      for (int j = 0; j < 8; ++j) {
        const int m = m0 + wr * 128 + j * 16 + c;
        if (m >= a.M) continue;
#pragma unroll
        for (int i = 0; i < 4; ++i) {
          const int n = n0 + wc * 128 + h * 64 + i * 16 + g * 4;
          if (n < a.N) epi_store<EPI_F32>(a, sub[i][j], m, n, 0);
        }
      }
  }
}

template <int PD>
__global__ void __launch_bounds__(NTHR, 1) gemm_tn4w4_kernel(g256::TnMulti t) {
  __shared__ __attribute__((aligned(16))) char q0[32768];
  __shared__ __attribute__((aligned(16))) char q1[32768];
  __shared__ __attribute__((aligned(16))) char q2[32768];
  __shared__ __attribute__((aligned(16))) char q3[32768];
  const int pos = xcd_remap(blockIdx.x, t.ntiles);
  const int id = t.tile0 + (t.use_perm ? (int)t.perm[pos] : pos);
  int p = 0;
  for (int q = 1; q < t.n; ++q)
    if (id >= t.d[q].start) p = q;
  const g256::TnDesc& d = t.d[p];
  GemmArgs a{};
  a.A = d.A; a.lda = d.lda;
  a.B = d.B; a.ldb = d.ldb;
  a.C = d.C; a.ldc = d.ldc;
  a.dbias = d.db;
  a.M = d.M; a.N = d.N; a.K = d.K;
  a.staged = d.staged;
  a.cmask = d.cmask;
  const int local = d.tiles ? (int)d.tiles[id - d.start] : id - d.start;
  const int ntn = (a.N + BN - 1) / BN;
  const int tm = local / ntn, tn = local % ntn;
  const int wc = __builtin_amdgcn_readfirstlane(threadIdx.x >> 6) & 1;
  const int m0 = tm * BM, n0 = tn * BN;
  const bool spread = d.tiles == nullptr && ntn >= 2;
  if (a.dbias != nullptr && (spread ? tn < 2 : tn == 0)) {
    if (!spread) {
      if (wc == 0) tile_body4<0x0F, PD>(a, m0, n0, q0, q1, q2, q3);
      else tile_body4<0xF0, PD>(a, m0, n0, q0, q1, q2, q3);
    } else if (tn == 0) {
      if (wc == 0) tile_body4<0x03, PD>(a, m0, n0, q0, q1, q2, q3);
      else tile_body4<0x0C, PD>(a, m0, n0, q0, q1, q2, q3);
    } else {
      if (wc == 0) tile_body4<0x30, PD>(a, m0, n0, q0, q1, q2, q3);
      else tile_body4<0xC0, PD>(a, m0, n0, q0, q1, q2, q3);
    }
  } else {
    tile_body4<0, PD>(a, m0, n0, q0, q1, q2, q3);
  }
}

}

bool launch_tn4w_multi(const g256::TnMulti& t, hipStream_t stream) {
  for (int i = 0; i < t.n; ++i) {
    const g256::TnDesc& d = t.d[i];
    if (d.K <= 0 || d.K % (2 * tn4w::BK) || d.M % 8 || d.N % 8 || d.lda % 8 || d.ldb % 8 ||
        ((unsigned long)d.A & 15) || ((unsigned long)d.B & 15))
      return false;
  }
  hipLaunchKernelGGL(tn4w::gemm_tn4w4_kernel<3>, dim3(t.ntiles), dim3(tn4w::NTHR), 0, stream, t);
  NF_HIP_CHECK(hipGetLastError());
  return true;
}

}
}
```

vi_normflows_amd/models/realnvp.py:

```python
from __future__ import annotations

import math
from dataclasses import dataclass, field

import torch

from ..ops import fused
from ..ops import gemm
from ..utils.config import KernelPaths
from ..utils.flat import FlatLayout, FlatParams
from .engine_core import FlatEngine, anneal_beta


@dataclass
class RealNVPConfig:
    dim: int = 784
    n_layers: int = 32
    hidden: int = 1024
    n_hidden: int = 2
    scale_bound: float = 1.0
    target: str = "banana"
    banana_sigma1: float = 1.0
    banana_sigma2: float = 0.5
    banana_bend: float = 0.5
    banana_pairing: str = "interleaved"
    gaussian_scale: float = 0.7
    learn_base: bool = True
    init_out_std: float = 1e-3
    anneal: str = "reference"
    anneal_iters: int = 10000
    k_align: int = 32
    paths: KernelPaths | None = None
    extra: dict = field(default_factory=dict)

    @property
    def half(self) -> int:
        assert self.dim % 2 == 0, "RealNVP needs an even dimension"
        return self.dim // 2

    @property
    def half_pad(self) -> int:
        a = max(1, self.k_align)
        return (self.half + a - 1) // a * a

    @property
    def out_pad(self) -> int:
        a = max(1, self.k_align)
        return (2 * self.half + a - 1) // a * a

    def n_params(self) -> int:
        Dh, H = self.half, self.hidden
        per = Dh * H + H + (self.n_hidden - 1) * (H * H + H) + H * 2 * Dh + 2 * Dh
        return self.n_layers * per + 2 * self.dim

    def flops_per_sample(self) -> float:
        Dh, H = self.half, self.hidden
        macs = Dh * H + (self.n_hidden - 1) * H * H + H * 2 * Dh
        return 6.0 * macs * self.n_layers


def _layer_shapes(cfg: RealNVPConfig, H: int | None = None):
    H = cfg.hidden if H is None else H
    dims = [cfg.half_pad] + [H] * cfg.n_hidden + [cfg.out_pad]
    return [(dims[i + 1], dims[i]) for i in range(len(dims) - 1)]


class RealNVPVI(FlatEngine):

    supports_forward_persist = True
    trace_forward, trace_backward = "flow_forward+elbo", "flow_backward"

    def __init__(self, cfg: RealNVPConfig, batch: int, device="cuda",
                 compute_dtype: torch.dtype | None = None, seed: int = 0, rank: int = 0,
                 lr: float = 1e-4, optimizer="adam", betas=(0.9, 0.999),
                 eps: float = 1e-8, weight_decay: float = 0.0, max_grad_norm: float = 0.0,
                 lr_warmup: float = 0.0):
        self.cfg = cfg
        self.B = int(batch)
        self.device = torch.device(device)
        if compute_dtype is None:
            compute_dtype = torch.bfloat16 if self.device.type == "cuda" else torch.float32
        self.cdt = compute_dtype
        self.seed = int(seed)
        self.rank = int(rank)
        self._init_core(optimizer, betas, eps, lr, weight_decay, max_grad_norm, lr_warmup)
        self.wgrad_fence_hook = None
        self.eps_override = None

        L = cfg.n_layers
        layout = FlatLayout()
        layout.add_unit([("base.mu", (cfg.dim,)), ("base.logvar", (cfg.dim,))])
        a = max(1, cfg.k_align)
        pad = self.device.type == "cuda" and self.cdt == torch.bfloat16
        self.Hp = (cfg.hidden + a - 1) // a * a if pad else cfg.hidden
        self.shapes = _layer_shapes(cfg, self.Hp)
        for l in range(L):
            ts = []
            for i, (o, inp) in enumerate(self.shapes):
                ts += [(f"l{l}.W{i}", (o, inp)), (f"l{l}.b{i}", (o,))]
            layout.add_unit(ts)
        self.layout = layout
        self.params = FlatParams(layout, self.device, self.cdt)
        self._alloc_state()
        self.beta = torch.ones((), dtype=torch.float32, device=self.device)
        self._alloc_workspace()
        self.init_params(seed)

    def _alloc_workspace(self):
        cfg, B, dev = self.cfg, self.B, self.device
        L, Dh, H, D = cfg.n_layers, cfg.half, self.Hp, cfg.dim
        f32 = torch.float32
        self.z0 = torch.empty(B, D, dtype=f32, device=dev)
        self.eps0 = torch.empty(B, D, dtype=f32, device=dev)
        self.Hs = torch.empty(L, B, Dh, dtype=f32, device=dev)
        Dp, Np = cfg.half_pad, cfg.out_pad
        self.Hbf = torch.empty(L, B, Dp, dtype=self.cdt, device=dev)
        self.Act = torch.empty(L, cfg.n_hidden, B, H, dtype=self.cdt, device=dev)
        self.Mk = None
        kp = cfg.paths if cfg.paths is not None else KernelPaths.from_env()
        if dev.type == "cuda" and H % 8 == 0:
            self.Mk = torch.empty(L, cfg.n_hidden, B, H // 8, dtype=torch.uint8, device=dev)
        self.mk_lanes_path = (self.Mk is not None and kp.relu_mask_lanes
                              and B % 256 == 0 and H % 256 == 0)
        self.mk_lanes = [False] * cfg.n_hidden
        self.ST = torch.empty(L, B, Np, dtype=self.cdt, device=dev)
        self.st = self.ST[0]
        self.dst2 = [torch.empty(B, Np, dtype=self.cdt, device=dev) for _ in range(2)]
        self.dst = self.dst2[0]
        self.dH2 = [[torch.empty(B, H, dtype=self.cdt, device=dev)
                     for _ in range(max(cfg.n_hidden, 1))] for _ in range(2)]
        self.dH = self.dH2[0]
        self.wgrad_defer = dev.type == "cuda" and kp.wgrad_defer
        self.cpl_fuse = self.wgrad_defer and kp.cpl_fuse
        self.cpl_xbf16 = kp.cpl_xbf16
        self.dstL = self.dHL = None
        kc = H if cfg.n_hidden else Dp
        self.cf_fuse = (dev.type == "cuda" and self.cdt == torch.bfloat16
                        and Dh % 8 == 0 and kc % 32 == 0
                        and kp.cpl_fwd_fuse)
        self.ldjp = None
        if self.cf_fuse:
            self.ldjp = torch.empty((Dh + 127) // 128, B, dtype=f32, device=dev)
        self.wt_dgrad = self.wgrad_defer and kp.dgrad_nt
        self.WT = None
        self._wt_plan = None
        self._wplan = None
        if self.wgrad_defer:
            self.dstL = torch.empty(L, B, Np, dtype=self.cdt, device=dev)
            self.dHL = torch.empty(L, max(cfg.n_hidden, 1), B, H, dtype=self.cdt, device=dev)
            self._wchunk = torch.cuda.get_device_properties(dev).multi_processor_count
        self.wgrad_stream = None
        if dev.type == "cuda" and kp.wgrad_stream:
            self.wgrad_stream = torch.cuda.Stream(device=dev)
        self._G = torch.zeros(L + 2, B, Dp, dtype=f32, device=dev)
        self.G = self._G[:, :, :Dh]
        self._rg_partial = None
        if dev.type == "cuda" and D % 4 == 0 and Dh % 4 == 0 and Dp % 4 == 0 and D <= 1024:
            self._rg_partial = torch.empty(512 * 2 * D, dtype=f32, device=dev)
        self.logq0 = torch.empty(B, dtype=f32, device=dev)
        self.ldj = torch.empty(B, dtype=f32, device=dev)
        self.logp = torch.empty(B, dtype=f32, device=dev)
        self.frow = torch.empty(B, dtype=f32, device=dev)
        self._target_params = None
        if cfg.target == "gaussian":
            m = torch.zeros(D, device=dev)
            iv = torch.full((D,), 1.0 / cfg.gaussian_scale ** 2, device=dev)
            self._target_params = torch.cat([m, iv]).contiguous()

    def h(self, i: int) -> torch.Tensor:
        Dh = self.cfg.half
        if i == 0:
            return self.z0[:, Dh:]
        if i == 1:
            return self.z0[:, :Dh]
        return self.Hs[i - 2]

    def _cpl_x(self, i: int, has_wt: bool) -> torch.Tensor:
        if i >= 1 and self.cpl_xbf16 and has_wt and self.cdt == torch.bfloat16:
            return self.Hbf[i - 1][:, :self.cfg.half]
        return self.h(i)

    def zK_halves(self):
        L = self.cfg.n_layers
        a, b = (L + 1, L) if (L + 1) % 2 == 1 else (L, L + 1)
        return self.h(a), self.h(b), a, b

    def init_params(self, seed: int = 0):
        g = torch.Generator(device="cpu").manual_seed(int(seed))
        P = self.params
        n_lin = len(self.shapes)
        Dh, No = self.cfg.half, 2 * self.cfg.half
        H, Hp = self.cfg.hidden, self.Hp
        for l in range(self.cfg.n_layers):
            for i, (o, inp) in enumerate(self.shapes):
                ro = H if i < n_lin - 1 else o
                ri = H if i > 0 else inp
                fan_in = Dh if i == 0 else ri
                std = math.sqrt(2.0 / fan_in) if i < n_lin - 1 else self.cfg.init_out_std
                W = torch.zeros(o, inp)
                b = torch.zeros(o)
                W[:ro, :ri] = torch.randn(ro, ri, generator=g) * std
                b[:ro] = torch.randn(ro, generator=g) * (0.01 if i < n_lin - 1
                                                         else self.cfg.init_out_std)
                if i == 0:
                    W[:, Dh:] = 0.0
                if i == n_lin - 1:
                    W[No:, :] = 0.0
                    b[No:] = 0.0
                P.p(f"l{l}.W{i}").copy_(W)
                P.p(f"l{l}.b{i}").copy_(b)
        P.p("base.mu").zero_()
        P.p("base.logvar").zero_()
        P.sync_compute()
        P.reset_optimizer_state()
        self.step_t.zero_()
        self.rng_offset.zero_()

    def _target_args(self):
        cfg = self.cfg
        if cfg.target == "banana":
            s1, s2 = cfg.banana_sigma1, cfg.banana_sigma2
            pairs = cfg.dim // 2
            cst = -pairs * (math.log(2 * math.pi) + math.log(s1) + math.log(s2))
            kind = fused.TARGET_BANANA_SPLIT if cfg.banana_pairing == "split" else fused.TARGET_BANANA
            return dict(kind=kind, params=None, p0=s1, p1=s2, p2=cfg.banana_bend,
                        cst=cst)
        if cfg.target == "gaussian":
            D, s = cfg.dim, cfg.gaussian_scale
            cst = -0.5 * D * math.log(2 * math.pi) - D * math.log(s)
            return dict(kind=fused.TARGET_GAUSSIAN, params=self._target_params, cst=cst)
        raise ValueError(cfg.target)

    def log_normalizer(self) -> float:
        return 0.0

    def _update_schedule(self):
        self._advance()
        if self.cfg.anneal == "reference":
            anneal_beta("reference", self.step_t, self.cfg.anneal_iters, self.beta)
        else:
            self.beta.fill_(1.0)

    def _mask_lanes(self):
        cfg = self.cfg
        self.mk_lanes = [False] * cfg.n_hidden
        if not (self.mk_lanes_path and gemm.backend() == "mfma" and self.cdt == torch.bfloat16):
            return
        wt = self.wt_dgrad and self.wgrad_stream is None
        for i in range(cfg.n_hidden):
            k_fwd, k_bwd = self.shapes[i][1], self.shapes[i + 1][0]
            self.mk_lanes[i] = gemm.mask_lanes_route(self.B, self.Hp, k_fwd, k_bwd, wt)

    def _conditioner_hidden(self, l: int, inp: torch.Tensor) -> torch.Tensor:
        P = self.params
        a = inp
        for i in range(self.cfg.n_hidden):
            out = self.Act[l, i]
            gemm.linear_fwd(a, P.c(f"l{l}.W{i}"), P.c(f"l{l}.b{i}"), out, relu=True,
                            mask_out=None if self.Mk is None else self.Mk[l, i],
                            mask_lanes=self.mk_lanes[i])
            a = out
        return a

    def _conditioner_fwd(self, l: int, inp: torch.Tensor) -> torch.Tensor:
        P = self.params
        nh = self.cfg.n_hidden
        a = self._conditioner_hidden(l, inp)
        st = self.ST[l]
        gemm.linear_fwd(a, P.c(f"l{l}.W{nh}"), P.c(f"l{l}.b{nh}"), st, relu=False)
        return st

    def forward(self):
        cfg, P = self.cfg, self.params
        Dh = cfg.half
        if self.eps_override is None:
            fused.reparam_sample(self.z0, mu=P.p("base.mu"), logvar=P.p("base.logvar"),
                                 seed=self.seed, offset=self.rng_offset, stream_id=self.rank,
                                 eps=self.eps0, zbf=self.Hbf[0], nbf=Dh, logq0=self.logq0)
        else:
            self._base_from_eps(self.eps_override)
        self._flow_layers()
        A, Bh, ia, ib = self.zK_halves()
        ta = self._target_args()
        fused.target_logp_grad(ta["kind"], A, Bh, gA=self.G[ia], gB=self.G[ib],
                               grad_accumulate=False, params=ta.get("params"), p0=ta.get("p0", 1.0),
                               p1=ta.get("p1", 1.0), p2=ta.get("p2", 0.0), cst=ta["cst"],
                               beta=self.beta, row_weight=1.0 / self.B, logq0=self.logq0,
                               ldj=self.ldj, logp_out=self.logp, frow_out=self.frow)
        torch.mean(self.frow, 0, out=self.loss)

    def _flow_layers(self):
        cfg, P = self.cfg, self.params
        L, nh = cfg.n_layers, cfg.n_hidden
        fuse = self.cf_fuse and gemm.backend() == "mfma"
        self._mask_lanes()
        for l in range(L):
            ybf = self.Hbf[l + 1] if l + 1 < L else None
            if fuse:
                a = self._conditioner_hidden(l, self.Hbf[l])
                gemm.linear_fwd_coupling(a, P.c(f"l{l}.W{nh}"), P.c(f"l{l}.b{nh}"), self.ST[l],
                                         self.h(l), self.h(l + 2), ybf, self.ldjp,
                                         ldj_init=(l == 0), scale=cfg.scale_bound)
                continue
            st = self._conditioner_fwd(l, self.Hbf[l])
            fused.coupling_fwd(st, self.h(l), self.h(l + 2), ybf=ybf, ssav=None,
                               ldj=self.ldj, scale=cfg.scale_bound, inverse=False,
                               ldj_init=(l == 0))
        if fuse:
            torch.sum(self.ldjp, 0, out=self.ldj)

    def _base_from_eps(self, eps: torch.Tensor):
        P, cfg = self.params, self.cfg
        lv = P.p("base.logvar")
        self.eps0.copy_(eps)
        self.z0.copy_(P.p("base.mu") + torch.exp(0.5 * lv) * eps)
        self.Hbf[0][:, :cfg.half].copy_(self.z0[:, :cfg.half].to(self.cdt))
        self.Hbf[0][:, cfg.half:].zero_()
        self.logq0.copy_(-0.5 * cfg.dim * math.log(2 * math.pi) - 0.5 * lv.sum()
                         - 0.5 * (eps * eps).sum(1))

    def _wgrad_plan(self):
        if self._wplan is None:
            cfg, P = self.cfg, self.params
            L, nh = cfg.n_layers, cfg.n_hidden
            items, layer_last = [], {}
            for l in range(L - 1, -1, -1):
                d = self.dstL[l]
                for i in range(nh, -1, -1):
                    inp = self.Act[l, i - 1] if i > 0 else self.Hbf[l]
                    items.append((d, inp, P.g(f"l{l}.W{i}"), P.g(f"l{l}.b{i}")))
                    if i > 0:
                        d = self.dHL[l, i - 1]
                layer_last[l] = len(items) - 1
            plan = gemm.WgradPlan(items)
            plan.layer_end = {l: plan.end_of(k) for l, k in layer_last.items()}
            self._wplan = plan
        return self._wplan

    def _weights_t(self):
        if self._wt_plan is None:
            from ..ops.layout import TransposePlan

            cfg, P = self.cfg, self.params
            Ws = [[P.c(f"l{l}.W{i}") for i in range(cfg.n_hidden + 1)]
                  for l in range(cfg.n_layers)]
            buf = torch.empty(sum(W.numel() for row in Ws for W in row), dtype=self.cdt,
                              device=self.device)
            self.WT, pairs, off = [], [], 0
            for row in Ws:
                out = []
                for W in row:
                    o, i = W.shape
                    Wt = buf[off:off + o * i].view(i, o)
                    off += o * i
                    out.append(Wt)
                    pairs.append((W, Wt))
                self.WT.append(out)
            self._wt_plan = TransposePlan(pairs)
        self._wt_plan.run()
        return self.WT

    def _backward_deferred(self):
        cfg, P = self.cfg, self.params
        L, nh = cfg.n_layers, cfg.n_hidden
        c = -1.0 / self.B
        plan = self._wgrad_plan()
        sched = gemm.WgradScheduler(plan, [(l + 1, plan.layer_end[l]) for l in range(L - 1, -1, -1)],
                                    self._wchunk, self.unit_ready_hook, self.wgrad_fence_hook)
        fuse = self.cpl_fuse

        def wgrad_ready(l):
            sched.ready(plan.layer_end[l], final=(l == 0))

        def cpl_bwd(l):
            fused.coupling_bwd(self.G[l + 2], self.ST[l][:, :cfg.half], self.h(l), self.dstL[l],
                               self.G[l], c=c, scale=cfg.scale_bound, gx_accumulate=False,
                               s_is_hat=True)

        WT = self._weights_t() if self.wt_dgrad else None
        if fuse:
            cpl_bwd(L - 1)
        for l in range(L - 1, -1, -1):
            if not fuse:
                cpl_bwd(l)
            d = self.dstL[l]
            for i in range(nh, -1, -1):
                if i > 0:
                    nd = self.dHL[l, i - 1]
                    gemm.linear_dgrad(d, P.c(f"l{l}.W{i}"), nd, relu_of=self.Act[l, i - 1],
                                      relu_bits=None if self.Mk is None else self.Mk[l, i - 1],
                                      Wt=None if WT is None else WT[l][i],
                                      bits_lanes=self.mk_lanes[i - 1])
                    d = nd
                elif fuse and l > 0:
                    xb = self._cpl_x(l - 1, WT is not None)
                    gin, gout = self._G[l + 1], self._G[l - 1][:, :cfg.half]
                    gemm.linear_dgrad_coupling(d, P.c(f"l{l}.W0"), gin,
                                               s_hat=self.ST[l - 1][:, :cfg.half],
                                               x=xb, dst=self.dstL[l - 1], gx=gout,
                                               scale=cfg.scale_bound, c=c,
                                               Wt=None if WT is None else WT[l][0])
                else:
                    gemm.linear_dgrad(d, P.c(f"l{l}.W0"), self._G[l + 1], accumulate=True)
            wgrad_ready(l)
        self._base_backward()
        self._mark_ready(0)

    def backward(self):
        if (self.wgrad_defer and self.wgrad_stream is None and gemm.backend() == "mfma"
                and self.cdt == torch.bfloat16):
            return self._backward_deferred()
        cfg, P = self.cfg, self.params
        L, nh = cfg.n_layers, cfg.n_hidden
        c = -1.0 / self.B
        side = self.wgrad_stream
        main = torch.cuda.current_stream(self.device) if side is not None else None
        done = [None, None]
        for l in range(L - 1, -1, -1):
            par = l % 2
            if done[par] is not None:
                main.wait_event(done[par])
            dst, dH = self.dst2[par], self.dH2[par]
            fused.coupling_bwd(self.G[l + 2], self.ST[l][:, :cfg.half], self.h(l), dst, self.G[l],
                               c=c, scale=cfg.scale_bound, gx_accumulate=False, s_is_hat=True)
            d = dst
            wg = []
            for i in range(nh, -1, -1):
                inp = self.Act[l, i - 1] if i > 0 else self.Hbf[l]
                wg.append((d, inp, P.g(f"l{l}.W{i}"), P.g(f"l{l}.b{i}")))
                if i > 0:
                    nd = dH[i - 1]
                    gemm.linear_dgrad(d, P.c(f"l{l}.W{i}"), nd, relu_of=self.Act[l, i - 1],
                                      relu_bits=None if self.Mk is None else self.Mk[l, i - 1],
                                      bits_lanes=self.mk_lanes[i - 1])
                    d = nd
                else:
                    gemm.linear_dgrad(d, P.c(f"l{l}.W0"), self._G[l + 1], accumulate=True)
            if side is not None:
                ready = torch.cuda.Event()
                ready.record(main)
                side.wait_event(ready)
                with torch.cuda.stream(side):
                    gemm.linear_wgrad_group(wg)
                    self._mark_ready(l + 1)
                    ev = torch.cuda.Event()
                    ev.record(side)
                done[par] = ev
            else:
                gemm.linear_wgrad_group(wg)
                self._mark_ready(l + 1)
        for ev in done:
            if ev is not None:
                main.wait_event(ev)
        self._base_backward()
        self._mark_ready(0)

    def _base_backward(self):
        cfg, P = self.cfg, self.params
        gmu, glv = P.g("base.mu"), P.g("base.logvar")
        if not cfg.learn_base:
            gmu.zero_()
            glv.zero_()
            return
        if self._rg_partial is not None:
            fused.reparam_grad(self.G[1], self.G[0], self.eps0, P.p("base.logvar"),
                               self._rg_partial, gmu, glv)
            return
        g0 = torch.cat([self.G[1], self.G[0]], 1)
        torch.sum(g0, 0, out=gmu)
        sig = torch.exp(0.5 * P.p("base.logvar"))
        torch.sum(g0 * self.eps0, 0, out=glv)
        glv.mul_(0.5 * sig).sub_(0.5)

    @torch.no_grad()
    def sample(self, n: int | None = None, offset: int = 10**9):
        n = n or self.B
        assert n <= self.B
        cfg, P = self.cfg, self.params
        Dh = cfg.half
        fused.reparam_sample(self.z0, mu=P.p("base.mu"), logvar=P.p("base.logvar"),
                             seed=self.seed + 1, offset_host=offset, stream_id=self.rank,
                             eps=self.eps0, zbf=self.Hbf[0], nbf=Dh, logq0=self.logq0)
        self._flow_layers()
        A, Bh, _, _ = self.zK_halves()
        z = torch.cat([A, Bh], 1)[:n].clone()
        logq = (self.logq0 - self.ldj)[:n].clone()
        return z, logq

    @torch.no_grad()
    def inverse(self, z: torch.Tensor):
        cfg = self.cfg
        n, D = z.shape
        assert D == cfg.dim and n <= self.B, (z.shape, self.B)
        Dh, L = cfg.half, cfg.n_layers
        A, Bh, ia, ib = self.zK_halves()
        A.zero_()
        Bh.zero_()
        A[:n].copy_(z[:, :Dh])
        Bh[:n].copy_(z[:, Dh:])
        top = self.Hbf[L - 1]
        top[:, Dh:].zero_()
        top[:, :Dh].copy_(self.h(L))
        fuse = self.cf_fuse and gemm.backend() == "mfma"
        P, nh = self.params, cfg.n_hidden
        self._mask_lanes()
        for l in range(L - 1, -1, -1):
            nxt = self.Hbf[l - 1] if l > 0 else None
            if fuse:
                a = self._conditioner_hidden(l, self.Hbf[l])
                gemm.linear_fwd_coupling(a, P.c(f"l{l}.W{nh}"), P.c(f"l{l}.b{nh}"), None,
                                         self.h(l + 2), self.h(l), nxt, self.ldjp,
                                         ldj_init=(l == L - 1), scale=cfg.scale_bound,
                                         inverse=True)
                continue
            st = self._conditioner_fwd(l, self.Hbf[l])
            fused.coupling_fwd(st, self.h(l + 2), self.h(l), ybf=nxt, ssav=None, ldj=self.ldj,
                               scale=cfg.scale_bound, inverse=True, ldj_init=(l == L - 1))
        if fuse:
            torch.sum(self.ldjp, 0, out=self.ldj)
        return self.z0[:n].clone(), self.ldj[:n].clone()

    @torch.no_grad()
    def log_prob(self, z: torch.Tensor) -> torch.Tensor:
        z0, ldj_inv = self.inverse(z)
        P = self.params
        mu, lv = P.p("base.mu"), P.p("base.logvar")
        q = (z0 - mu) * torch.exp(-0.5 * lv)
        lq0 = -0.5 * self.cfg.dim * math.log(2 * math.pi) - 0.5 * lv.sum() - 0.5 * (q * q).sum(1)
        return lq0 + ldj_inv
```

vi_normflows_amd/ops/gemm.py:

```python
from __future__ import annotations

import contextlib
import threading

import torch

_state = threading.local()


@contextlib.contextmanager
def oracle():
    prev = getattr(_state, "oracle", False)
    _state.oracle = True
    try:
        yield
    finally:
        _state.oracle = prev


def backend() -> str:
    return "oracle" if getattr(_state, "oracle", False) else "mfma"


def _mfma_ok(*ts) -> bool:
    if getattr(_state, "oracle", False):
        return False
    cuda = [t for t in ts if t is not None and t.is_cuda]
    if not cuda:
        return False
    bad = [t.dtype for t in cuda if t.dtype != torch.bfloat16]
    if bad:
        raise TypeError(f"GPU GEMM operands must be bf16 for the MFMA kernels (got {bad[0]}); "
                        "use `with ops.gemm.oracle():` for an explicit torch reference")
    return True


LANES_OK, LANES_SHAPE, LANES_KERNEL = 0, 1, 2


def mask_lanes_route(M: int, N: int, K_fwd: int, K_bwd: int, bwd_wt: bool) -> bool:
    from ._ext import native

    return native().gemm_mask_lanes_route(int(M), int(N), int(K_fwd), int(K_bwd),
                                          bool(bwd_wt)) == LANES_OK


def linear_fwd(x: torch.Tensor, W: torch.Tensor, b: torch.Tensor | None, out: torch.Tensor,
               relu: bool = False, mask_out: torch.Tensor | None = None,
               mask_lanes: bool = False) -> torch.Tensor:
    if _mfma_ok(x, W):
        from ._ext import native

        if mask_lanes and relu and mask_out is not None:
            rc = native().gemm_nt(x, W, b, out, 1, mask_out, True)
            if rc == LANES_OK:
                return out
            if rc != LANES_SHAPE:
                raise RuntimeError("linear_fwd: lane-private mask asked for on a product that "
                                   "runs the 128x128 kernel (see ops.gemm.mask_lanes_route)")
        native().gemm_nt(x, W, b, out, 1 if relu else 0, mask_out if relu else None)
        return out
    if b is not None:
        torch.addmm(b, x, W.t(), out=out)
    else:
        torch.mm(x, W.t(), out=out)
    if relu:
        out.relu_()
    return out


def linear_dgrad(dy: torch.Tensor, W: torch.Tensor, out: torch.Tensor,
                 relu_of: torch.Tensor | None = None, accumulate: bool = False,
                 relu_bits: torch.Tensor | None = None,
                 Wt: torch.Tensor | None = None, bits_lanes: bool = False) -> torch.Tensor:
    if _mfma_ok(dy, W):
        from ._ext import native

        if relu_bits is not None and bits_lanes:
            rc = native().gemm_nn(dy, W, None, out, bool(accumulate), relu_bits, Wt, True)
            if rc == LANES_OK:
                return out
            if rc != LANES_SHAPE:
                raise RuntimeError("linear_dgrad: lane-private bits on a product that runs the "
                                   "128x128 kernel (see ops.gemm.mask_lanes_route)")
        if relu_bits is not None:
            native().gemm_nn(dy, W, None, out, bool(accumulate), relu_bits, Wt)
        else:
            native().gemm_nn(dy, W, relu_of, out, bool(accumulate), None, Wt)
        return out
    if dy.is_cuda and out.dtype != dy.dtype:
        r = torch.mm(dy, W, out_dtype=out.dtype)
    else:
        r = torch.mm(dy, W)
    if relu_of is not None:
        r = r * (relu_of > 0)
    if accumulate:
        out.add_(r)
    else:
        out.copy_(r)
    return out


def linear_fwd_coupling(h: torch.Tensor, W: torch.Tensor, b: torch.Tensor | None,
                        st: torch.Tensor | None, x: torch.Tensor, y: torch.Tensor,
                        ybf: torch.Tensor | None, ldjp: torch.Tensor, ldj_init: bool,
                        scale: float, inverse: bool = False) -> None:
    Dh = x.shape[1]
    if _mfma_ok(h, W):
        from ._ext import native

        native().gemm_nt_cpl(h, W, b, st, x, y, ybf, ldjp, bool(ldj_init), float(scale),
                             bool(inverse))
        return
    o = h.float() @ W.float().t()
    if b is not None:
        o = o + b.float()
    o = o.to(st.dtype).float()
    sh, t = o[:, :Dh], o[:, Dh:2 * Dh]
    s = scale * torch.tanh(sh)
    yv = (x - t) * torch.exp(-s) if inverse else x * torch.exp(s) + t
    if st is not None:
        st[:, :Dh].copy_(sh)
    y.copy_(yv)
    if ybf is not None:
        ybf[:, :Dh].copy_(yv)
        ybf[:, Dh:].zero_()
    part = -s.sum(1) if inverse else s.sum(1)
    if ldj_init:
        ldjp.zero_()
        ldjp[0].copy_(part)
    else:
        ldjp[0].add_(part)


def linear_dgrad_coupling(dy: torch.Tensor, W: torch.Tensor, G: torch.Tensor, s_hat: torch.Tensor,
                          x: torch.Tensor, dst: torch.Tensor, gx: torch.Tensor, scale: float,
                          c: float, Wt: torch.Tensor | None = None) -> None:
    if _mfma_ok(dy, W):
        from ._ext import native

        native().gemm_nn_cpl(dy, W, G, s_hat, x, dst, gx, float(scale), float(c), Wt)
        return
    Dh = x.shape[1]
    gy = (G.float() + (dy.float() @ W.float()))[:, :Dh]
    s = scale * torch.tanh(s_hat[:, :Dh].float())
    es = torch.exp(s)
    ds = (gy * x * es + c) * (scale - s * s / scale)
    dst[:, :Dh].copy_(ds)
    dst[:, Dh:2 * Dh].copy_(gy)
    dst[:, 2 * Dh:].zero_()
    gx.copy_(gy * es)


def linear_wgrad_group(items) -> None:
    items = list(items)
    if items and all(_mfma_ok(dy, x) for dy, x, _, _ in items):
        from ._ext import native

        for c in range(0, len(items), 4):
            ch = items[c:c + 4]
            native().gemm_tn_group([i[0] for i in ch], [i[1] for i in ch], [i[2] for i in ch],
                                   [i[3] for i in ch], [None] * len(ch), [None] * len(ch))
        return
    for dy, x, dW, db in items:
        linear_wgrad(dy, x, dW, db)


def linear_wgrad(dy: torch.Tensor, x: torch.Tensor, dW: torch.Tensor,
                 db: torch.Tensor | None) -> None:
    if _mfma_ok(dy, x):
        from ._ext import native

        native().gemm_tn(dy, x, dW, db)
        return
    if dy.is_cuda and dW.dtype != dy.dtype:
        dW.copy_(torch.mm(dy.t(), x, out_dtype=dW.dtype))
    else:
        torch.mm(dy.t(), x, out=dW)
    if db is not None:
        torch.sum(dy, 0, dtype=db.dtype, out=db)


def wgrad_tiles(M: int, N: int) -> int:
    return ((M + 255) // 256) * ((N + 255) // 256)


class WgradPlan:

    MAX_PROBLEMS = 40

    def __init__(self, items, f8_scales: torch.Tensor | None = None, f8_idx=None):
        self.items = [tuple(i) + (None, None) if len(i) == 4 else tuple(i) for i in items]
        self.f8 = f8_scales is not None
        self.f8_scales = f8_scales
        self.f8_idx = [tuple(int(v) for v in t) for t in f8_idx] if self.f8 else None
        self._part = None
        if self.f8:
            assert len(self.f8_idx) == len(self.items)
            n_db = sum(int(it[0].shape[1]) for it in self.items if it[3] is not None)
            self._part = torch.empty(8 * max(n_db, 1), dtype=torch.float32,
                                     device=self.items[0][0].device)
        self.tiles = [wgrad_tiles(it[0].shape[1], it[1].shape[1]) if it[4] is None else
                      int(it[4].numel()) for it in self.items]
        self.starts = [0]
        for t in self.tiles:
            self.starts.append(self.starts[-1] + t)
        self.total = self.starts[-1]

    def end_of(self, idx: int) -> int:
        return self.starts[idx + 1]

    def run(self, tile0: int, ntiles: int) -> None:
        import bisect

        if ntiles <= 0:
            return
        end = tile0 + ntiles
        assert 0 <= tile0 and end <= self.total, (tile0, ntiles, self.total)
        first = bisect.bisect_right(self.starts, tile0) - 1
        last = bisect.bisect_left(self.starts, end) - 1
        if self.f8:
            self._run_f8(tile0, end, first, last)
            return
        if not all(_mfma_ok(it[0], it[1]) for it in self.items[first:last + 1]):
            for p in range(first, last + 1):
                if tile0 < self.starts[p + 1] <= end:
                    dy, x, dW, db, _, cm = self.items[p]
                    linear_wgrad(dy, x, dW, db)
                    if cm is not None:
                        dW.mul_(cm)
            return
        from ._ext import native

        t = tile0
        while t < end:
            p0 = bisect.bisect_right(self.starts, t) - 1
            p1 = min(last, p0 + self.MAX_PROBLEMS - 1)
            stop = min(end, self.starts[p1 + 1])
            ch = self.items[p0:p1 + 1]
            masked = any(i[4] is not None or i[5] is not None for i in ch)
            native().gemm_tn_multi([i[0] for i in ch], [i[1] for i in ch], [i[2] for i in ch],
                                   [i[3] for i in ch], t - self.starts[p0], stop - t,
                                   [i[4] for i in ch] if masked else [],
                                   [i[5] for i in ch] if masked else [])
            t = stop


    def _f8_deq(self, p: int):
        dy, x = self.items[p][0], self.items[p][1]
        sa, sb = self.f8_idx[p]
        return dy.float() * self.f8_scales[sa], x.float() * self.f8_scales[sb]

    def _run_f8(self, tile0: int, end: int, first: int, last: int) -> None:
        import bisect

        done = [p for p in range(first, last + 1) if tile0 < self.starts[p + 1] <= end]
        if getattr(_state, "oracle", False) or not self.items[first][0].is_cuda:
            for p in done:
                dy, x = self._f8_deq(p)
                _, _, dW, db, _, cm = self.items[p]
                dW.copy_(dy.t() @ x)
                if cm is not None:
                    dW.mul_(cm)
                if db is not None:
                    db.copy_(dy.sum(0))
            return
        from ._ext import native

        t = tile0
        while t < end:
            p0 = bisect.bisect_right(self.starts, t) - 1
            p1 = min(last, p0 + self.MAX_PROBLEMS - 1)
            stop = min(end, self.starts[p1 + 1])
            ch = self.items[p0:p1 + 1]
            idx = self.f8_idx[p0:p1 + 1]
            native().gemm_tn_multi_f8([i[0] for i in ch], [i[1] for i in ch], [i[2] for i in ch],
                                      [None] * len(ch), t - self.starts[p0], stop - t,
                                      [i[4] for i in ch], [i[5] for i in ch], self.f8_scales,
                                      [a for a, _ in idx], [b for _, b in idx])
            t = stop
        dbs = [p for p in done if self.items[p][3] is not None]
        for k in range(0, len(dbs), self.MAX_PROBLEMS):
            ps = dbs[k:k + self.MAX_PROBLEMS]
            native().fp8_colsum([self.items[p][0] for p in ps], [self.items[p][3] for p in ps],
                                self.f8_scales, [self.f8_idx[p][0] for p in ps], self._part)


class WgradScheduler:

    def __init__(self, plan: WgradPlan, unit_ends, chunk: int, hook=None, fence=None):
        self.plan, self.unit_ends, self.chunk, self.hook = plan, list(unit_ends), int(chunk), hook
        self.fence = fence
        self.launched = 0
        self._next = 0

    def ready(self, avail_end: int, final: bool = False) -> None:
        while avail_end - self.launched >= self.chunk or (final and self.launched < avail_end):
            n = min(self.chunk, avail_end - self.launched)
            if self.fence is not None:
                self.fence()
            self.plan.run(self.launched, n)
            self.launched += n
            while (self._next < len(self.unit_ends)
                   and self.unit_ends[self._next][1] <= self.launched):
                if self.hook is not None:
                    self.hook(self.unit_ends[self._next][0])
                self._next += 1
```

vi_normflows_amd/utils/config.py:

```python
from __future__ import annotations

import copy
import json
from dataclasses import asdict, dataclass, field, fields, is_dataclass
from pathlib import Path


@dataclass
class RunConfig:
    name: str = "custom"
    task: str = "flow_vi"
    device: str = "auto"
    seed: int = 0
    iters: int = 1000
    lr: float = 1e-3
    optimizer: str = "adam"
    schedule: str = "none"
    batch: int = 256
    log_every: int = 100
    ckpt_every: int = 0
    out_dir: str = "runs"
    target: str = "U1"
    flow: str = "planar"
    K: int = 8
    dim: int = 2
    hidden: int = 64
    n_hidden: int = 2
    dim_z: int = 40
    lr_warmup: float = 0.0
    max_grad_norm: float = 0.0
    pairing: str = "split"
    extra: dict = field(default_factory=dict)

    def override(self, items: list[str]) -> "RunConfig":
        c = copy.deepcopy(self)
        names = {f.name: f for f in fields(c)}
        for it in items:
            if "=" not in it:
                raise ValueError(f"override must be key=value: {it}")
            k, v = it.split("=", 1)
            try:
                val = json.loads(v)
            except json.JSONDecodeError:
                val = v
            if k.startswith("extra."):
                c.extra[k[6:]] = val
            elif k in names:
                setattr(c, k, type(getattr(c, k))(val) if getattr(c, k) is not None and
                        not isinstance(getattr(c, k), dict) else val)
            else:
                raise KeyError(f"unknown config key {k}")
        return c

    def validate(self) -> "RunConfig":
        from ..inference.annealing import SCHEDULES

        if self.schedule not in SCHEDULES:
            raise ValueError(f"unknown schedule {self.schedule!r}; expected one of {sorted(SCHEDULES)}")
        if self.pairing not in ("split", "interleaved"):
            raise ValueError(f"unknown pairing {self.pairing!r}; expected 'split' or 'interleaved'")
        if self.lr_warmup < 0 or self.max_grad_norm < 0:
            raise ValueError("lr_warmup and max_grad_norm must be >= 0")
        return self

    def to_dict(self) -> dict:
        return asdict(self)

    def save(self, path) -> None:
        Path(path).parent.mkdir(parents=True, exist_ok=True)
        Path(path).write_text(json.dumps(self.to_dict(), indent=2))


PRESETS: dict[str, RunConfig] = {
    "config1_two_moons_cpu": RunConfig(name="config1_two_moons_cpu", task="flow_vi", device="cpu",
                                       target="U1", flow="planar", K=16, dim=2, iters=10000,
                                       lr=1e-2, batch=256, optimizer="adam"),
    "config2_realnvp8": RunConfig(name="config2_realnvp8", task="realnvp_vi", device="cuda",
                                  K=8, dim=784, hidden=1024, batch=65536, iters=200, lr=1e-3,
                                  lr_warmup=100.0, schedule="none", pairing="split"),
    "config3_realnvp32_dp8": RunConfig(name="config3_realnvp32_dp8", task="realnvp_vi",
                                       device="cuda", K=32, dim=784, hidden=1024, batch=65536,
                                       iters=200, lr=1e-3, lr_warmup=100.0, schedule="none",
                                       pairing="split"),
    "config3_realnvp32_annealed": RunConfig(name="config3_realnvp32_annealed", task="realnvp_vi",
                                            device="cuda", K=32, dim=784, hidden=1024,
                                            batch=65536, iters=2000, lr=1e-4, lr_warmup=100.0,
                                            schedule="reference", pairing="split"),
    "config4_iaf10_vae": RunConfig(name="config4_iaf10_vae", task="iaf_vae", device="cuda", K=10,
                                   dim=3072, hidden=1024, dim_z=256, batch=1024, iters=200,
                                   lr=3e-4),
    "config5_maf64": RunConfig(name="config5_maf64", task="maf_density", device="cuda", K=64,
                               dim=1024, hidden=1024, n_hidden=1, batch=8192, iters=200, lr=1e-4,
                               extra={"precision": "fp8", "impl": "engine"}),
    "mnist_planar_vae": RunConfig(name="mnist_planar_vae", task="planar_vae", device="auto", K=4,
                                  dim=784, hidden=64, n_hidden=3, dim_z=40, batch=128,
                                  iters=10000, lr=1e-3, schedule="reference"),
}


def load(spec: str | None, overrides: list[str] | None = None) -> RunConfig:
    if spec is None:
        cfg = RunConfig()
    elif spec in PRESETS:
        cfg = copy.deepcopy(PRESETS[spec])
    else:
        p = Path(spec)
        text = p.read_text()
        if p.suffix in (".yaml", ".yml"):
            import yaml

            data = yaml.safe_load(text)
        else:
            data = json.loads(text)
        base = copy.deepcopy(PRESETS.get(data.get("preset", ""), RunConfig()))
        data.pop("preset", None)
        cfg = base.override([f"{k}={json.dumps(v)}" for k, v in data.items()
                             if k != "extra"])
        cfg.extra.update(data.get("extra", {}))
    return cfg.override(overrides or []).validate()


def rank_seed(seed: int, rank: int) -> int:
    return (int(seed) * 1_000_003 + 7919 * int(rank)) % (2 ** 31 - 1)


def is_config(obj) -> bool:
    return is_dataclass(obj)


@dataclass
class KernelPaths:
    wgrad_defer: bool = True
    dgrad_nt: bool = True
    cpl_fuse: bool = True
    cpl_fwd_fuse: bool = True
    cpl_xbf16: bool = True
    relu_mask_lanes: bool = True
    wgrad_stream: bool = False
    maf_fuse: bool = True
    fp8_dgrad: bool = True
    fp8_wgrad: bool = True
    maf_bf16_state: bool = False
    made_fused: bool = True

    @classmethod
    def from_env(cls) -> "KernelPaths":
        import os

        p = cls()
        spec = os.environ.get("VINF_KERNEL_PATHS", "").strip()
        if not spec:
            return p
        names = {f.name for f in fields(cls)}
        for item in spec.split(","):
            k, _, v = item.strip().partition("=")
            if k not in names:
                raise ValueError(f"VINF_KERNEL_PATHS: unknown path {k!r} (known: {sorted(names)})")
            setattr(p, k, v.strip().lower() not in ("0", "false", "off", "no"))
        return p
```

Measured before the change: 2.018 million samples/s.

## Fold ragged 784-row wgrad tail into fat 288-row tiles with optional K-split

Adds a 'fat' weight-gradient GEMM kernel that covers M in (256,288] with one extra 16-row wave fragment per tile. The ragged last 16 rows of the 784-row output (784 = 3*256+16) no longer need a mostly empty extra 256-row tile. The remainder rows are folded into the last full tile, the regular tiles are rescheduled, and the fat tiles run as a tail at the end of the wgrad schedule. When the fat tiles fill less than half of the CUs, the K dimension is split in two, with a slab buffer and a combine kernel reducing the halves. The cost is more register and LDS pressure per block, an extra combine launch, and the tail work being deferred to the final step.

After: 2.034 million samples/s (median of 6 runs). About the same (+0.8%).

```diff
diff --git a/csrc/bindings/gemm_ops.cpp b/csrc/bindings/gemm_ops.cpp
--- a/csrc/bindings/gemm_ops.cpp
+++ b/csrc/bindings/gemm_ops.cpp
@@ -357,6 +357,52 @@
   gemm_tn_multi_impl(dy, x, dW, db, tile0, ntiles, tiles, cmask, nullptr, {}, {});
 }
 
+void gemm_tn_fat(at::TensorList dy, at::TensorList x, at::TensorList dW,
+                 const c10::List<c10::optional<at::Tensor>>& db, int64_t tile0, int64_t ntiles,
+                 const c10::optional<at::Tensor>& slab) {
+  const size_t n = dy.size();
+  TORCH_CHECK(n >= 1 && n <= 40 && x.size() == n && dW.size() == n && db.size() == n,
+              "gemm_tn_fat: 1..40 problems with matching lists");
+  const bool split = slab && slab->defined();
+  std::vector<NfTnProblem> pr(n);
+  long total = 0;
+  for (size_t p = 0; p < n; ++p) {
+    chk_mat(dy[p], "dy", at::kBFloat16);
+    chk_mat(x[p], "x", at::kBFloat16);
+    chk_mat(dW[p], "dW", at::kFloat);
+    const int K = dy[p].size(0), M = dy[p].size(1), N = x[p].size(1);
+    TORCH_CHECK(x[p].size(0) == K, "batch mismatch");
+    TORCH_CHECK(dW[p].size(0) == M && dW[p].size(1) == N, "dW shape");
+    TORCH_CHECK(M > 256 && M <= 288 && M % 8 == 0 && N % 8 == 0 && N >= 8,
+                "gemm_tn_fat: 256 < M <= 288, M % 8, N % 8 required");
+    TORCH_CHECK(K > 0 && K % (split ? 256 : 128) == 0,
+                "gemm_tn_fat: K % 128 == 0 (K % 256 == 0 when split along K) required");
+    TORCH_CHECK(ld2(dy[p]) < (1L << 31) && ld2(x[p]) < (1L << 31) && ld2(dW[p]) < (1L << 31),
+                "leading dimensions must fit in int32");
+    float* dbp = nullptr;
+    const c10::optional<at::Tensor> b = db.get(p);
+    if (b && b->defined()) {
+      TORCH_CHECK(b->is_cuda() && b->scalar_type() == at::kFloat && b->numel() == M &&
+                      b->is_contiguous(), "db");
+      dbp = b->data_ptr<float>();
+    }
+    pr[p] = NfTnProblem{dy[p].data_ptr(), ld2(dy[p]), x[p].data_ptr(), ld2(x[p]),
+                        dW[p].data_ptr<float>(), ld2(dW[p]), dbp, M, N, K};
+    total += (N + 255) / 256;
+  }
+  TORCH_CHECK(tile0 >= 0 && ntiles >= 1 && tile0 + ntiles <= total, "tile range outside the ",
+              total, " fat tiles of the problem list");
+  float* sp = nullptr;
+  if (split) {
+    TORCH_CHECK(slab->is_cuda() && slab->scalar_type() == at::kFloat && slab->is_contiguous() &&
+                    slab->numel() >= ntiles * 74016L &&
+                    reinterpret_cast<uintptr_t>(slab->data_ptr()) % 16 == 0,
+                "gemm_tn_fat: slab must be a 16-B aligned fp32 GPU buffer of ntiles * 74016");
+    sp = slab->data_ptr<float>();
+  }
+  nf_launch_tn4w_fat((int)n, pr.data(), (int)tile0, (int)ntiles, split ? 1 : 0, sp, cur_stream());
+}
+
 void gemm_tn_multi_f8(at::TensorList dy, at::TensorList x, at::TensorList dW,
                       const c10::List<c10::optional<at::Tensor>>& db, int64_t tile0,
                       int64_t ntiles, const c10::List<c10::optional<at::Tensor>>& tiles,
@@ -1060,6 +1106,7 @@
   m.def("gemm_tn(Tensor dy, Tensor x, Tensor(a!) dW, Tensor(b!)? db) -> ()");
   m.def("gemm_tn_group(Tensor[] dy, Tensor[] x, Tensor(a!)[] dW, Tensor(b!)?[] db, Tensor?[] skip, Tensor?[] cmask) -> ()");
   m.def("gemm_tn_multi(Tensor[] dy, Tensor[] x, Tensor(a!)[] dW, Tensor(b!)?[] db, int tile0, int ntiles, Tensor?[] tiles, Tensor?[] cmask) -> ()");
+  m.def("gemm_tn_fat(Tensor[] dy, Tensor[] x, Tensor(a!)[] dW, Tensor(b!)?[] db, int tile0, int ntiles, Tensor(c!)? slab) -> ()");
   m.def("gemm_tn_multi_layout(Tensor[] dy, Tensor[] x, Tensor(a!)[] dW, Tensor(b!)?[] db, int tile0, int ntiles, int layout) -> ()");
   m.def("fp8_colsum(Tensor[] q, Tensor(a!)[] out, Tensor scales, int[] sidx, Tensor(b!) part) -> ()");
   m.def("gemm_tn_multi_f8(Tensor[] dy, Tensor[] x, Tensor(a!)[] dW, Tensor(b!)?[] db, int tile0, int ntiles, Tensor?[] tiles, Tensor?[] cmask, Tensor scales, int[] sa_idx, int[] sb_idx) -> ()");
@@ -1088,6 +1135,7 @@
   m.impl("gemm_tn", &gemm_tn);
   m.impl("gemm_tn_group", &gemm_tn_group);
   m.impl("gemm_tn_multi", &gemm_tn_multi);
+  m.impl("gemm_tn_fat", &gemm_tn_fat);
   m.impl("gemm_tn_multi_f8", &gemm_tn_multi_f8);
   m.impl("fp8_colsum", &fp8_colsum);
   m.impl("gemm_tn_multi_layout", &gemm_tn_multi_layout);
diff --git a/csrc/include/launchers.h b/csrc/include/launchers.h
--- a/csrc/include/launchers.h
+++ b/csrc/include/launchers.h
@@ -181,6 +181,8 @@
                                   long ldc, long slab_stride, float* dbias, int M, int N, int K,
                                   int splits, hipStream_t stream);
 int nf_gemm256_tiles(int M, int N);
+void nf_launch_tn4w_fat(int nprob, const NfTnProblem* pr, int tile0, int ntiles, int ksplit,
+                        float* slab, hipStream_t stream);
 void nf_launch_gemm256_tn_multi(int nprob, const NfTnProblem* pr, int tile0, int ntiles,
                                 hipStream_t stream, const float* f8_scales = nullptr,
                                 int layout = 0);
diff --git a/csrc/include/tn_multi.h b/csrc/include/tn_multi.h
--- a/csrc/include/tn_multi.h
+++ b/csrc/include/tn_multi.h
@@ -22,13 +22,19 @@
   int n, tile0, ntiles, use_perm;
   unsigned short perm[TN_PERM_MAX];
   const float* scales;
+  float* slab;
+  int ksplit;
 };
 static_assert(sizeof(TnMulti) <= 4096, "TnMulti must fit the 4 KiB kernarg segment");
+
+constexpr int TN_FAT_ROWS = 288;
+constexpr long TN_FAT_SLAB = (long)TN_FAT_ROWS * 256 + TN_FAT_ROWS;
 
 }
 
 
 bool launch_tn4w_multi(const g256::TnMulti& t, hipStream_t stream);
+bool launch_tn4w_fat(const g256::TnMulti& t, hipStream_t stream);
 
 }
 }
diff --git a/csrc/kernels/gemm_tn4w.hip b/csrc/kernels/gemm_tn4w.hip
--- a/csrc/kernels/gemm_tn4w.hip
+++ b/csrc/kernels/gemm_tn4w.hip
@@ -1,4 +1,5 @@
 
+#include "launchers.h"
 #include "tn_multi.h"
 
 #include <cstdlib>
@@ -38,11 +39,64 @@
   }
 }
 
+__device__ __forceinline__ int x_swz(int k) { return ((k >> 3) & 1) << 1; }
+
+__device__ __forceinline__ unsigned stage_x_voff(long ld, int col0, int cols_total, int lane) {
+  const int kr = lane >> 2;
+  const int lc = (lane & 3) ^ x_swz(kr);
+  int gm = col0 + lc * 8;
+  gm = gm < cols_total ? gm : cols_total - 8;
+  return (unsigned)((kr * ld + gm) * 2);
+}
+__device__ __forceinline__ void stage_x(const bf16_t* __restrict__ base, long ld, unsigned voff,
+                                        int k0, char* dst, int piece) {
+  const char* row = (const char*)base + (long)(k0 + piece * 16) * ld * 2;
+  const unsigned lds = (unsigned)(unsigned long)(LDS_AS char*)(dst + piece * 1024);
+  asm volatile("s_mov_b32 m0, %2\n\tglobal_load_lds_dwordx4 %0, %1"
+               :: "v"(voff), "s"(row), "s"(lds) : "memory", "m0");
+}
+__device__ __forceinline__ v8s read_frag_x(const char* img, int r0, int lane) {
+  const int i = lane & 15, g = lane >> 4;
+  const int col = r0 + 4 * (i & 3);
+  const int chunk = col >> 3, sub = (col >> 2) & 1;
+  v8s out;
+#pragma unroll
+  for (int h = 0; h < 2; ++h) {
+    const int k = 8 * g + 4 * h + (i >> 2);
+    const LDS_AS v4s* p =
+        (const LDS_AS v4s*)(img + k * 64 + ((chunk ^ x_swz(k)) << 4) + sub * 8);
+    const v4s t = __builtin_amdgcn_ds_read_tr16_b64_v4i16((LDS_AS v4s*)p);
+    if (h == 0) {
+      out[0] = t[0]; out[1] = t[1]; out[2] = t[2]; out[3] = t[3];
+    } else {
+      out[4] = t[0]; out[5] = t[1]; out[6] = t[2]; out[7] = t[3];
+    }
+  }
+  return out;
+}
+
+__device__ __forceinline__ void mfma_acc_last(v4f& acc, const v8s& a, const v8s& b) {
+  asm volatile("v_mfma_f32_16x16x32_bf16 %0, %1, %2, %0\n\ts_nop 7\n\ts_nop 7"
+               : "+a"(acc) : "v"(a), "v"(b));
+}
+__device__ __forceinline__ void mfma_accv_last(v4f& acc, const v8s& a, const v8s& b) {
+  asm volatile("v_mfma_f32_16x16x32_bf16 %0, %1, %2, %0\n\ts_nop 7\n\ts_nop 7"
+               : "+v"(acc) : "v"(a), "v"(b));
+}
+
+template <int N>
+__device__ __forceinline__ void wait_vm() {
+  asm volatile("s_waitcnt vmcnt(%0)" :: "n"(N) : "memory");
+}
+
 __device__ __forceinline__ void mfma_acc(v4f& acc, const v8s& a, const v8s& b) {
   asm volatile("v_mfma_f32_16x16x32_bf16 %0, %1, %2, %0" : "+a"(acc) : "v"(a), "v"(b));
 }
-
-template <int DBM, int PD>
+__device__ __forceinline__ void mfma_accv(v4f& acc, const v8s& a, const v8s& b) {
+  asm volatile("v_mfma_f32_16x16x32_bf16 %0, %1, %2, %0" : "+v"(acc) : "v"(a), "v"(b));
+}
+
+template <int DBM, int PD, bool FAT = false, bool XD = false, bool XDB = false>
 __device__ __forceinline__ void tile_body4(const GemmArgs& a, int m0, int n0, char* q0, char* q1,
                                            char* q2, char* q3) {
   constexpr int BK4 = 32, HALF4 = 128 * BK4 * 2;
@@ -58,8 +112,12 @@
     constexpr int Q = decltype(q_c)::value;
     return Q == 0 ? q0 : Q == 1 ? q1 : Q == 2 ? q2 : q3;
   };
+  constexpr int NDMA = 8 + ((FAT && XD) ? 1 : 0);
+  unsigned xvoff = 0;
+  if constexpr (FAT && XD) xvoff = stage_x_voff(a.lda, m0 + 256, a.M, lane);
   auto issue = [&](int t, auto q_c) {
     stage<8>(sbase, sld, scol0, stot, t * BK4, stp(q_c) + wave * HALF4, lane);
+    if constexpr (FAT && XD) stage_x(a.A, a.lda, xvoff, t * BK4, stp(q_c) + 4 * HALF4, wr);
   };
   v4f acc[8][8];
 #pragma unroll
@@ -70,6 +128,14 @@
 #pragma unroll
   for (int j = 0; j < 8; ++j) dbs[j] = 0.f;
   v8s fa[8], fb0[8], fb1[8];
+  v4f accx[FAT ? 8 : 1];
+  v8s fx0, fx1;
+  float dbx = 0.f;
+  if constexpr (FAT) {
+#pragma unroll
+    for (int i = 0; i < 8; ++i) accx[i] = (v4f){0.f, 0.f, 0.f, 0.f};
+  }
+  auto rd_x = [&](auto q_c) { return read_frag_x(stp(q_c) + 4 * HALF4, wr * 16, lane); };
   auto rd_a = [&](auto q_c, int j) { return read_frag<false>(stp(q_c) + wr * HALF4, j * 16, 0, lane); };
   auto rd_b = [&](auto q_c, v8s (&fb)[8]) {
     const char* st = stp(q_c) + (2 + wc) * HALF4;
@@ -80,7 +146,10 @@
   auto mfma_j = [&](const v8s (&fb)[8], auto qn_c, auto rd_c, auto j_c) {
     constexpr int j = decltype(j_c)::value;
 #pragma unroll
-    for (int i = 0; i < 8; ++i) mfma_acc(acc[i][j], fb[i], fa[j]);
+    for (int i = 0; i < 8; ++i) {
+      if constexpr (FAT && !decltype(rd_c)::value) mfma_acc_last(acc[i][j], fb[i], fa[j]);
+      else mfma_acc(acc[i][j], fb[i], fa[j]);
+    }
     if constexpr ((DBM >> j) & 1) {
       typedef __bf16 v2bf __attribute__((ext_vector_type(2)));
       const v2bf one = {(__bf16)1.0f, (__bf16)1.0f};
@@ -110,23 +179,24 @@
   issue(1, std::integral_constant<int, 1>{});
   if constexpr (PD == 3) {
     issue(2, std::integral_constant<int, 2>{});
-    asm volatile("s_waitcnt vmcnt(16)" ::: "memory");
+    wait_vm<2 * NDMA>();
   } else {
-    asm volatile("s_waitcnt vmcnt(8)" ::: "memory");
+    wait_vm<NDMA>();
   }
   __builtin_amdgcn_s_barrier();
 #pragma unroll
   for (int j = 0; j < 8; ++j) fa[j] = rd_a(std::integral_constant<int, 0>{}, j);
   rd_b(std::integral_constant<int, 0>{}, fb0);
-  auto ktile = [&](int t, auto q_c, const v8s (&fbc)[8], v8s (&fbn)[8], auto w2_c, auto next_c,
-                   auto issue_c) {
+  if constexpr (FAT) fx0 = rd_x(std::integral_constant<int, 0>{});
+  auto ktile = [&](int t, auto q_c, const v8s (&fbc)[8], v8s (&fbn)[8], const v8s& fxc, v8s& fxn,
+                   auto w2_c, auto next_c, auto issue_c) {
     constexpr int Q = decltype(q_c)::value;
     using QN = std::integral_constant<int, (Q + 1) & 3>;
     using QI = std::integral_constant<int, (Q + PD) & 3>;
     asm volatile("s_waitcnt lgkmcnt(0)" ::: "memory");
     if constexpr (decltype(next_c)::value) {
-      if constexpr (PD == 3 && decltype(w2_c)::value) asm volatile("s_waitcnt vmcnt(8)" ::: "memory");
-      else asm volatile("s_waitcnt vmcnt(0)" ::: "memory");
+      if constexpr (PD == 3 && decltype(w2_c)::value) wait_vm<NDMA>();
+      else wait_vm<0>();
     }
     __builtin_amdgcn_sched_barrier(0);
 #ifndef NF_PROBE_NOBAR
@@ -140,9 +210,27 @@
 #endif
     if constexpr (decltype(next_c)::value)
       fbn[0] = read_frag<false>(stp(QN{}) + (2 + wc) * HALF4, 0, 0, lane);
+    if constexpr (FAT && decltype(next_c)::value) fxn = rd_x(QN{});
     fbn_p = fbn;
     __builtin_amdgcn_sched_barrier(0);
     kstep_from1(fbc, QN{}, next_c);
+    if constexpr (FAT) {
+#pragma unroll
+      for (int i = 0; i < 8; ++i) {
+        if constexpr (!decltype(next_c)::value) mfma_accv_last(accx[i], fbc[i], fxc);
+        else mfma_accv(accx[i], fbc[i], fxc);
+      }
+      if constexpr (XDB) {
+        typedef __bf16 v2bf __attribute__((ext_vector_type(2)));
+        const v2bf one = {(__bf16)1.0f, (__bf16)1.0f};
+#pragma unroll
+        for (int e = 0; e < 4; ++e) {
+          const unsigned w = (unsigned)(unsigned short)fxc[2 * e] |
+                             ((unsigned)(unsigned short)fxc[2 * e + 1] << 16);
+          dbx = __builtin_amdgcn_fdot2_f32_bf16(__builtin_bit_cast(v2bf, w), one, dbx, false);
+        }
+      }
+    }
   };
   using Q0 = std::integral_constant<int, 0>;
   using Q1 = std::integral_constant<int, 1>;
@@ -150,20 +238,20 @@
   using Q3 = std::integral_constant<int, 3>;
   int t = 0;
   for (; t + 4 < nkt; t += 4) {
-    ktile(t, Q0{}, fb0, fb1, T{}, T{}, T{});
-    ktile(t + 1, Q1{}, fb1, fb0, T{}, T{}, T{});
-    ktile(t + 2, Q2{}, fb0, fb1, T{}, T{}, T{});
-    ktile(t + 3, Q3{}, fb1, fb0, T{}, T{}, T{});
+    ktile(t, Q0{}, fb0, fb1, fx0, fx1, T{}, T{}, T{});
+    ktile(t + 1, Q1{}, fb1, fb0, fx1, fx0, T{}, T{}, T{});
+    ktile(t + 2, Q2{}, fb0, fb1, fx0, fx1, T{}, T{}, T{});
+    ktile(t + 3, Q3{}, fb1, fb0, fx1, fx0, T{}, T{}, T{});
   }
   if constexpr (PD == 3) {
-    ktile(t, Q0{}, fb0, fb1, T{}, T{}, T{});
-    ktile(t + 1, Q1{}, fb1, fb0, T{}, T{}, F{});
+    ktile(t, Q0{}, fb0, fb1, fx0, fx1, T{}, T{}, T{});
+    ktile(t + 1, Q1{}, fb1, fb0, fx1, fx0, T{}, T{}, F{});
   } else {
-    ktile(t, Q0{}, fb0, fb1, F{}, T{}, T{});
-    ktile(t + 1, Q1{}, fb1, fb0, F{}, T{}, T{});
-  }
-  ktile(t + 2, Q2{}, fb0, fb1, F{}, T{}, F{});
-  ktile(t + 3, Q3{}, fb1, fb0, F{}, F{}, F{});
+    ktile(t, Q0{}, fb0, fb1, fx0, fx1, F{}, T{}, T{});
+    ktile(t + 1, Q1{}, fb1, fb0, fx1, fx0, F{}, T{}, T{});
+  }
+  ktile(t + 2, Q2{}, fb0, fb1, fx0, fx1, F{}, T{}, F{});
+  ktile(t + 3, Q3{}, fb1, fb0, fx1, fx0, F{}, F{}, F{});
 
   const int g = lane >> 4, c = lane & 15;
   if constexpr (DBM != 0) {
@@ -177,6 +265,13 @@
       if (g == 0 && m < a.M) a.dbias[m] = v;
     }
   }
+  if constexpr (FAT && XDB) {
+    float v = dbx;
+    v += __shfl_xor(v, 16);
+    v += __shfl_xor(v, 32);
+    const int m = m0 + 256 + wr * 16 + c;
+    if (g == 0 && m < a.M) a.dbias[m] = v;
+  }
   __builtin_amdgcn_sched_barrier(0);
   asm volatile("s_nop 7\n\ts_nop 7" ::: "memory");
   __builtin_amdgcn_sched_barrier(0);
@@ -203,6 +298,30 @@
           if (n < a.N) epi_store<EPI_F32>(a, sub[i][j], m, n, 0);
         }
       }
+  }
+  if constexpr (FAT) {
+    const int mx = m0 + 256 + wr * 16;
+    GemmArgs ax = a;
+    ax.M = a.M < mx + 16 ? a.M : mx + 16;
+#pragma unroll
+    for (int h = 0; h < 2; ++h) {
+      v4f sub[4][2];
+#pragma unroll
+      for (int i = 0; i < 4; ++i) {
+        sub[i][0] = accx[4 * h + i];
+        sub[i][1] = (v4f){0.f, 0.f, 0.f, 0.f};
+      }
+      if (a.staged)
+        epi_tile_staged<EPI_F32, 2>(ax, sub, mx, n0 + wc * 128 + h * 64, 0, region + h * 16384,
+                                    lane);
+      else if (mx + c < a.M) {
+#pragma unroll
+        for (int i = 0; i < 4; ++i) {
+          const int n = n0 + wc * 128 + h * 64 + i * 16 + g * 4;
+          if (n < a.N) epi_store<EPI_F32>(a, sub[i][0], mx + c, n, 0);
+        }
+      }
+    }
   }
 }
 
@@ -248,7 +367,161 @@
   }
 }
 
-}
+template <int PD>
+__global__ void __launch_bounds__(NTHR, 1) gemm_tn4wf_kernel(g256::TnMulti t) {
+  constexpr int STG = 32768 + 2048;
+  __shared__ __attribute__((aligned(16))) char q0[STG];
+  __shared__ __attribute__((aligned(16))) char q1[STG];
+  __shared__ __attribute__((aligned(16))) char q2[STG];
+  __shared__ __attribute__((aligned(16))) char q3[STG];
+  const int pos = xcd_remap(blockIdx.x, gridDim.x);
+  const int half = pos >= t.ntiles ? 1 : 0;
+  const int off = pos - half * t.ntiles;
+  const int id = t.tile0 + off;
+  int p = 0;
+  for (int q = 1; q < t.n; ++q)
+    if (id >= t.d[q].start) p = q;
+  const g256::TnDesc& d = t.d[p];
+  GemmArgs a{};
+  a.A = d.A; a.lda = d.lda;
+  a.B = d.B; a.ldb = d.ldb;
+  a.C = d.C; a.ldc = d.ldc;
+  a.dbias = d.db;
+  a.M = d.M; a.N = d.N; a.K = d.K;
+  a.staged = d.staged;
+  const int tn = id - d.start;
+  const int n0 = tn * BN;
+  if (t.ksplit) {
+    a.K = d.K >> 1;
+    if (half) {
+      a.A += (long)a.K * a.lda;
+      a.B += (long)a.K * a.ldb;
+      float* s = t.slab + (long)off * g256::TN_FAT_SLAB;
+      a.C = s - n0;
+      a.ldc = 256;
+      a.staged = 1;
+      if (a.dbias != nullptr) a.dbias = s + g256::TN_FAT_ROWS * 256;
+    }
+  }
+  const int wc = __builtin_amdgcn_readfirstlane(threadIdx.x >> 6) & 1;
+  if (a.dbias != nullptr && tn == 0) {
+    if (wc == 0) tile_body4<0x0F, PD, true, true, true>(a, 0, n0, q0, q1, q2, q3);
+    else tile_body4<0xF0, PD, true, false, false>(a, 0, n0, q0, q1, q2, q3);
+  } else {
+    if (wc == 0) tile_body4<0, PD, true, true, false>(a, 0, n0, q0, q1, q2, q3);
+    else tile_body4<0, PD, true, false, false>(a, 0, n0, q0, q1, q2, q3);
+  }
+}
+
+__global__ void __launch_bounds__(256) tn4wf_combine_kernel(g256::TnMulti t) {
+  const int off = blockIdx.x;
+  const int id = t.tile0 + off;
+  int p = 0;
+  for (int q = 1; q < t.n; ++q)
+    if (id >= t.d[q].start) p = q;
+  const g256::TnDesc& d = t.d[p];
+  const int tn = id - d.start;
+  const int n0 = tn * BN;
+  const float* s = t.slab + (long)off * g256::TN_FAT_SLAB;
+  const int r0 = blockIdx.y * 32;
+  const int n = n0 + (threadIdx.x & 63) * 4;
+  if (n < d.N) {
+#pragma unroll
+    for (int it = 0; it < 8; ++it) {
+      const int m = r0 + it * 4 + (threadIdx.x >> 6);
+      if (m >= d.M) break;
+      const float4 v = *reinterpret_cast<const float4*>(s + m * 256 + (n - n0));
+      float* cp = d.C + (long)m * d.ldc + n;
+      if (d.staged) {
+        float4 o = *reinterpret_cast<float4*>(cp);
+        o.x += v.x; o.y += v.y; o.z += v.z; o.w += v.w;
+        *reinterpret_cast<float4*>(cp) = o;
+      } else {
+        cp[0] += v.x; cp[1] += v.y; cp[2] += v.z; cp[3] += v.w;
+      }
+    }
+  }
+  if (d.db != nullptr && tn == 0 && threadIdx.x < 32) {
+    const int m = r0 + threadIdx.x;
+    if (m < d.M) d.db[m] += s[g256::TN_FAT_ROWS * 256 + m];
+  }
+}
+
+}
+
+static_assert(g256::TN_FAT_SLAB == 74016, "the bindings size the slab by this figure");
+
+bool launch_tn4w_fat(const g256::TnMulti& t, hipStream_t stream) {
+  if (t.n <= 0 || t.ntiles <= 0 || t.use_perm) return false;
+  if (t.ksplit && t.slab == nullptr) return false;
+  for (int i = 0; i < t.n; ++i) {
+    const g256::TnDesc& d = t.d[i];
+    if (d.M <= 256 || d.M > g256::TN_FAT_ROWS || d.K <= 0 ||
+        d.K % ((t.ksplit ? 4 : 2) * tn4w::BK) || d.M % 8 || d.N % 8 || d.lda % 8 || d.ldb % 8 ||
+        ((unsigned long)d.A & 15) || ((unsigned long)d.B & 15) || d.tiles != nullptr ||
+        d.cmask != nullptr)
+      return false;
+  }
+  hipLaunchKernelGGL(tn4w::gemm_tn4wf_kernel<3>, dim3(t.ntiles * (t.ksplit ? 2 : 1)),
+                     dim3(tn4w::NTHR), 0, stream, t);
+  NF_HIP_CHECK(hipGetLastError());
+  if (t.ksplit) {
+    hipLaunchKernelGGL(tn4w::tn4wf_combine_kernel, dim3(t.ntiles, g256::TN_FAT_ROWS / 32),
+                       dim3(256), 0, stream, t);
+    NF_HIP_CHECK(hipGetLastError());
+  }
+  return true;
+}
+
+}
+}
+
+void nf_launch_tn4w_fat(int nprob, const NfTnProblem* pr, int tile0, int ntiles, int ksplit,
+                        float* slab, hipStream_t stream) {
+  using namespace nf::gemm;
+  if (ntiles <= 0) return;
+  g256::TnMulti t{};
+  int base = 0;
+  for (int p = 0; p < nprob; ++p) {
+    const NfTnProblem& q = pr[p];
+    const int tiles = (q.N + 255) / 256;
+    if (base + tiles > tile0 && base < tile0 + ntiles) {
+      if (t.n >= g256::TN_MULTI_MAX) {
+        fprintf(stderr, "vinf: tn4w_fat: more than %d problems in one launch\n",
+                g256::TN_MULTI_MAX);
+        abort();
+      }
+      g256::TnDesc& d = t.d[t.n++];
+      d.A = (const nf::bf16_t*)q.dy; d.lda = (int)q.lddy;
+      d.B = (const nf::bf16_t*)q.x; d.ldb = (int)q.ldx;
+      d.C = q.dW; d.ldc = (int)q.lddw;
+      d.db = q.db;
+      d.M = q.M; d.N = q.N; d.K = q.K;
+      d.start = base;
+      GemmArgs a{};
+      a.C = q.dW; a.ldc = q.lddw; a.N = q.N;
+      d.staged = staged_ok(a, EPI_F32);
+    }
+    base += tiles;
+  }
+  if (tile0 < 0 || tile0 + ntiles > base || t.n == 0) {
+    fprintf(stderr, "vinf: tn4w_fat: tile range [%d, %d) outside the %d tiles\n", tile0,
+            tile0 + ntiles, base);
+    abort();
+  }
+  t.tile0 = tile0;
+  t.ntiles = ntiles;
+  t.ksplit = ksplit ? 1 : 0;
+  t.slab = slab;
+  if (!launch_tn4w_fat(t, stream)) {
+    fprintf(stderr, "vinf: tn4w_fat: every problem needs 256 < M <= 288, M / N / ld %% 8, 16-B "
+                    "aligned operands and K %% %d == 0\n", ksplit ? 256 : 128);
+    abort();
+  }
+}
+
+namespace nf {
+namespace gemm {
 
 bool launch_tn4w_multi(const g256::TnMulti& t, hipStream_t stream) {
   for (int i = 0; i < t.n; ++i) {
diff --git a/vi_normflows_amd/models/realnvp.py b/vi_normflows_amd/models/realnvp.py
--- a/vi_normflows_amd/models/realnvp.py
+++ b/vi_normflows_amd/models/realnvp.py
@@ -145,6 +145,9 @@
         self.WT = None
         self._wt_plan = None
         self._wplan = None
+        self.wgrad_fold = kp.wgrad_fold and B % 128 == 0
+        self.wgrad_fold_split = kp.wgrad_fold_split
+        self._wplan_fold = None
         if self.wgrad_defer:
             self.dstL = torch.empty(L, B, Np, dtype=self.cdt, device=dev)
             self.dHL = torch.empty(L, max(cfg.n_hidden, 1), B, H, dtype=self.cdt, device=dev)
@@ -319,7 +322,16 @@
         self.logq0.copy_(-0.5 * cfg.dim * math.log(2 * math.pi) - 0.5 * lv.sum()
                          - 0.5 * (eps * eps).sum(1))
 
-    def _wgrad_plan(self):
+    def _wgrad_plan(self, fold: bool = False):
+        if fold and self._wplan_fold is None:
+            base = self._wgrad_plan()
+            plan = gemm.WgradPlan([it[:4] for it in base.items], fold=True,
+                                  split=None if self.wgrad_fold_split else False,
+                                  cus=self._wchunk)
+            plan.layer_end = {l: plan.end_of(k) for l, k in base.layer_last.items()}
+            self._wplan_fold = plan
+        if fold:
+            return self._wplan_fold
         if self._wplan is None:
             cfg, P = self.cfg, self.params
             L, nh = cfg.n_layers, cfg.n_hidden
@@ -334,6 +346,7 @@
                 layer_last[l] = len(items) - 1
             plan = gemm.WgradPlan(items)
             plan.layer_end = {l: plan.end_of(k) for l, k in layer_last.items()}
+            plan.layer_last = layer_last
             self._wplan = plan
         return self._wplan
 
@@ -364,7 +377,9 @@
         cfg, P = self.cfg, self.params
         L, nh = cfg.n_layers, cfg.n_hidden
         c = -1.0 / self.B
-        plan = self._wgrad_plan()
+        fold = (self.wgrad_fold and self.unit_ready_hook is None
+                and self.wgrad_fence_hook is None)
+        plan = self._wgrad_plan(fold)
         sched = gemm.WgradScheduler(plan, [(l + 1, plan.layer_end[l]) for l in range(L - 1, -1, -1)],
                                     self._wchunk, self.unit_ready_hook, self.wgrad_fence_hook)
         fuse = self.cpl_fuse
diff --git a/vi_normflows_amd/ops/gemm.py b/vi_normflows_amd/ops/gemm.py
--- a/vi_normflows_amd/ops/gemm.py
+++ b/vi_normflows_amd/ops/gemm.py
@@ -185,13 +185,56 @@
     return ((M + 255) // 256) * ((N + 255) // 256)
 
 
+FAT_SLAB = 288 * 256 + 288
+
+
+def wgrad_fold_rows(M: int):
+    q, r = divmod(int(M), 256)
+    if q < 1 or r == 0 or r > 32:
+        return None
+    return 256 * (q - 1), 256 + r
+
+
 class WgradPlan:
 
     MAX_PROBLEMS = 40
 
-    def __init__(self, items, f8_scales: torch.Tensor | None = None, f8_idx=None):
+    def __init__(self, items, f8_scales: torch.Tensor | None = None, f8_idx=None,
+                 fold: bool = False, split: bool | None = None, cus: int | None = None):
         self.items = [tuple(i) + (None, None) if len(i) == 4 else tuple(i) for i in items]
         self.f8 = f8_scales is not None
+        self.fat_items, self.fat_tiles, self.fat_starts, self.part = [], 0, [0], None
+        self.split, self._slab = False, None
+        if fold:
+            assert not self.f8, "the folded form is bf16 only"
+            reg, self.part = [], []
+            for dy, x, dW, db, tl, cm in self.items:
+                rows = wgrad_fold_rows(dy.shape[1]) if tl is None and cm is None else None
+                if rows is None:
+                    self.part.append((len(reg), None))
+                    reg.append((dy, x, dW, db, tl, cm))
+                    continue
+                m0 = rows[0]
+                ri = None
+                if m0 > 0:
+                    ri = len(reg)
+                    reg.append((dy[:, :m0], x, dW[:m0], None if db is None else db[:m0],
+                                None, None))
+                self.part.append((ri, len(self.fat_items)))
+                self.fat_items.append((dy[:, m0:], x, dW[m0:], None if db is None else db[m0:]))
+                self.fat_starts.append(self.fat_starts[-1] + (int(x.shape[1]) + 255) // 256)
+            self.items = reg
+            self.fat_tiles = self.fat_starts[-1]
+            if self.fat_tiles:
+                dev = self.fat_items[0][0].device
+                if cus is None:
+                    cus = (torch.cuda.get_device_properties(dev).multi_processor_count
+                           if dev.type == "cuda" else 256)
+                self.split = (split is not False and 2 * self.fat_tiles <= int(cus)
+                              and all(int(i[0].shape[0]) % 256 == 0 for i in self.fat_items))
+                if self.split and dev.type == "cuda":
+                    self._slab = torch.empty(self.fat_tiles * FAT_SLAB, dtype=torch.float32,
+                                             device=dev)
         self.f8_scales = f8_scales
         self.f8_idx = [tuple(int(v) for v in t) for t in f8_idx] if self.f8 else None
         self._part = None
@@ -208,7 +251,31 @@
         self.total = self.starts[-1]
 
     def end_of(self, idx: int) -> int:
+        if self.part is not None:
+            ri = self.part[idx][0]
+            if ri is None:
+                ri = next((r for r, _ in self.part[idx + 1:] if r is not None), len(self.items))
+                return self.starts[ri]
+            idx = ri
         return self.starts[idx + 1]
+
+    def run_tail(self) -> None:
+        if not self.fat_items:
+            return
+        if not all(_mfma_ok(it[0], it[1]) for it in self.fat_items):
+            for dy, x, dW, db in self.fat_items:
+                linear_wgrad(dy, x, dW, db)
+            return
+        from ._ext import native
+
+        for p0 in range(0, len(self.fat_items), self.MAX_PROBLEMS):
+            ch = self.fat_items[p0:p0 + self.MAX_PROBLEMS]
+            t0, t1 = self.fat_starts[p0], self.fat_starts[p0 + len(ch)]
+            slab = None
+            if self.split:
+                slab = self._slab[t0 * FAT_SLAB:t1 * FAT_SLAB]
+            native().gemm_tn_fat([i[0] for i in ch], [i[1] for i in ch], [i[2] for i in ch],
+                                 [i[3] for i in ch], 0, t1 - t0, slab)
 
     def run(self, tile0: int, ntiles: int) -> None:
         import bisect
@@ -293,6 +360,7 @@
         self.fence = fence
         self.launched = 0
         self._next = 0
+        self._tail_pending = plan.fat_tiles > 0
 
     def ready(self, avail_end: int, final: bool = False) -> None:
         while avail_end - self.launched >= self.chunk or (final and self.launched < avail_end):
@@ -301,8 +369,17 @@
                 self.fence()
             self.plan.run(self.launched, n)
             self.launched += n
-            while (self._next < len(self.unit_ends)
-                   and self.unit_ends[self._next][1] <= self.launched):
-                if self.hook is not None:
-                    self.hook(self.unit_ends[self._next][0])
-                self._next += 1
+            self._fire()
+        if final and self._tail_pending:
+            if self.fence is not None:
+                self.fence()
+            self.plan.run_tail()
+            self._tail_pending = False
+            self._fire()
+
+    def _fire(self) -> None:
+        while (not self._tail_pending and self._next < len(self.unit_ends)
+               and self.unit_ends[self._next][1] <= self.launched):
+            if self.hook is not None:
+                self.hook(self.unit_ends[self._next][0])
+            self._next += 1
diff --git a/vi_normflows_amd/utils/config.py b/vi_normflows_amd/utils/config.py
--- a/vi_normflows_amd/utils/config.py
+++ b/vi_normflows_amd/utils/config.py
@@ -131,6 +131,8 @@
 @dataclass
 class KernelPaths:
     wgrad_defer: bool = True
+    wgrad_fold: bool = True
+    wgrad_fold_split: bool = True
     dgrad_nt: bool = True
     cpl_fuse: bool = True
     cpl_fwd_fuse: bool = True
```
